# klausondrag/FOSVOS

Hardware: AMD Instinct MI355X
Metric: online fine-tune frames/sec (854x480) (higher is better)
Workload: dtype bf16; 1 GPU; OSVOS_VGG train_online one-shot fine-tune: 1x3x480x854 frame per step, fwd + class-balanced BCE + bwd, fused SGD step every 5 steps (BASELINE.json configs[1]); batch=1, avg_grad_every_n=5, activations=bf16 NHWC, fp32 accumulate, fp32 master weights, parallelism=single GPU

## Files before the change

### fosvos_amd/csrc/conv_igemm.hip

```cpp
#include <stdlib.h>

#include "common.hpp"

using namespace fosvos;

namespace {

constexpr unsigned kReluAfterAdd = 0x100u;
constexpr unsigned kSubsample2 = 0x200u;
constexpr unsigned kNoSplitK = 0x400u;

struct ConvArgs {
    const uint16_t *x;
    const uint16_t *w;
    const float *bias;
    const uint16_t *relu_src;
    const uint8_t *relu_bits;
    const uint16_t *addend;
    void *y;
    uint16_t *y_pool;
    const uint16_t *unpool_g;
    int N, H, W, Cin, Cout, Co_pad;
    int tiles_x, tiles_y;
    unsigned flags;
    int swizzle;
    int k_splits;
    int chunks_per_split;
    float *partial;
    unsigned m_ncb, m_nt, m_tx, m_ty;
    int n_t;
#ifdef FOSVOS_STAMP
    unsigned long long *stamps;
#endif
};

#ifdef FOSVOS_STAMP
unsigned long long *g_stamps = nullptr;
#define FOSVOS_STAMP_AT(i)                                                                               \
    if (a.stamps && threadIdx.x == 0)                                                                    \
        a.stamps[((((int64_t)blockIdx.z * gridDim.y + blockIdx.y) * gridDim.x + blockIdx.x) << 4) + (i)] = \
            __builtin_amdgcn_s_memtime();
#define FOSVOS_STAMP_RT(i)                                                                               \
    if (a.stamps && threadIdx.x == 0)                                                                    \
        a.stamps[((((int64_t)blockIdx.z * gridDim.y + blockIdx.y) * gridDim.x + blockIdx.x) << 4) + (i)] = \
            __builtin_amdgcn_s_memrealtime();
#else
#define FOSVOS_STAMP_AT(i)
#define FOSVOS_STAMP_RT(i)
#endif

__device__ __forceinline__ unsigned fast_div(unsigned n, unsigned d, unsigned m) { return m ? __umulhi(n, m) : n / d; }
unsigned recip_mul(int64_t n_max, int64_t d) {
    return (d >= 2 && n_max * d < (int64_t(1) << 32)) ? (unsigned)((int64_t(1) << 32) / d + 1) : 0u;
}

template <int TH_, int TW_, int BN_, int WM_, int WN_>
struct Tile {
    static constexpr int TH = TH_, TW = TW_, BN = BN_, WM = WM_, WN = WN_;
    static constexpr int BM = TH * TW;
    static constexpr int HALO_W = TW + 2, HALO_H = TH + 2;
    static constexpr int NPIX = HALO_W * HALO_H;
    static constexpr int NPIX8 = (NPIX + 7) / 8 * 8;
    static constexpr int NPIX_PAD = (NPIX + 15) / 16 * 16;
    static constexpr int WAVE_M = BM / WM, WAVE_N = BN / WN;
    static constexpr int MF = WAVE_M / 16, NF = WAVE_N / 16;
    static constexpr int A_SLOTS = 4 * NPIX_PAD;
    static constexpr int B_SLOTS = 36 * BN;
    static constexpr int NT = 64 * WM * WN;
    static constexpr int A_IT = (NPIX8 * 4 + NT - 1) / NT;
    static constexpr int B_IT = (B_SLOTS + NT - 1) / NT;
    static constexpr int OUT_LD = BN + 8;
    static constexpr int LDS_MAIN = (A_SLOTS + B_SLOTS) * 16;
    static constexpr int LDS_OUT = BM * OUT_LD * 2;
    static constexpr int LDS_BYTES = LDS_MAIN > LDS_OUT ? LDS_MAIN : LDS_OUT;
#ifndef FOSVOS_MID_WPE
#define FOSVOS_MID_WPE 3
#endif
    static constexpr int WPE = (BM >= 256 || BN < 64) ? 2 : FOSVOS_MID_WPE;
    static_assert(WM * WN == 4 || WM * WN == 8, "4 or 8 waves per workgroup");
    static_assert(TW % 16 == 0 && WAVE_M % 16 == 0 && WAVE_N % 16 == 0, "fragment alignment");
    static_assert(BM % WM == 0 && BN % WN == 0, "wave split");
};

template <int MF, int NF>
struct TapPlan {
    static constexpr int rows_b = MF / 2 > 0 ? MF / 2 : 1;
    static constexpr int per_row = (NF + rows_b - 1) / rows_b;
    static constexpr int nb(int i) {
        const int left = NF - i * per_row;
        return left <= 0 ? 0 : (left < per_row ? left : per_row);
    }
};
template <int MF, int NF, int I, bool NEXT, int V>
__device__ __forceinline__ void sched_row() {
    if constexpr (I < MF) {
        __builtin_amdgcn_sched_group_barrier(0x008, NF, 0);
        if constexpr (NEXT) __builtin_amdgcn_sched_group_barrier(0x100, 1 + TapPlan<MF, NF>::nb(I), 0);
        constexpr int rows_v = V < MF ? V : MF;
        constexpr int nv = I < MF - rows_v ? 0 : (I == MF - 1 ? V - (rows_v - 1) : 1);
        if constexpr (nv > 0) __builtin_amdgcn_sched_group_barrier(0x020, nv, 0);
    }
}
template <int MF, int NF, bool NEXT, int V>
__device__ __forceinline__ void sched_tap() {
    static_assert(MF <= 8, "sched_tap rows");
    sched_row<MF, NF, 0, NEXT, V>(); sched_row<MF, NF, 1, NEXT, V>(); sched_row<MF, NF, 2, NEXT, V>();
    sched_row<MF, NF, 3, NEXT, V>(); sched_row<MF, NF, 4, NEXT, V>(); sched_row<MF, NF, 5, NEXT, V>();
    sched_row<MF, NF, 6, NEXT, V>(); sched_row<MF, NF, 7, NEXT, V>();
}

template <class T, bool OUT_F32, bool UNPOOL = false>
__global__ __launch_bounds__(T::NT) __attribute__((amdgpu_waves_per_eu(2, T::WPE))) void k_conv3x3_igemm(const ConvArgs a) {
    extern __shared__ __attribute__((aligned(16))) uint4 smem[];
    uint4 *sA = smem;
    uint4 *sB = smem + T::A_SLOTS;
#ifdef FOSVOS_IGEMM_PRIO
    __builtin_amdgcn_s_setprio(FOSVOS_IGEMM_PRIO);
#endif

    const int tid = threadIdx.x, lane = tid & 63;
    const int wave = __builtin_amdgcn_readfirstlane(tid >> 6);
    const int wm = wave / T::WN, wn = wave % T::WN;
    int t = blockIdx.x;
    int cb = blockIdx.y;
    if (a.swizzle) {
        const int n_wg = gridDim.x, n_cb = a.Cout / T::BN, n_t = a.n_t;
        const int q8 = n_wg >> 3, r8 = n_wg & 7, xcd = t & 7;
        const int swz = (xcd < r8 ? xcd * (q8 + 1) : r8 * (q8 + 1) + (xcd - r8) * q8) + (t >> 3);
        if (a.swizzle == 1) { t = fast_div(swz, n_cb, a.m_ncb); cb = swz - t * n_cb; }
        else { cb = fast_div(swz, n_t, a.m_nt); t = swz - cb * n_t; }
    }
    const int t_row = fast_div(t, a.tiles_x, a.m_tx);
    const int tx_i = t - t_row * a.tiles_x;
    const int n = fast_div(t_row, a.tiles_y, a.m_ty);
    const int ty_i = t_row - n * a.tiles_y;
    const int y0 = ty_i * T::TH, x0 = tx_i * T::TW;
    const int n0 = cb * T::BN;
    const int H = a.H, W = a.W, Cin = a.Cin;
    const int n_chunks = Cin >> 5;
    const uint16_t *xn = a.x + (int64_t)n * H * W * Cin;

    int a_goff[T::A_IT];
    int a_slot[T::A_IT];
#pragma unroll
    for (int it = 0; it < T::A_IT; ++it) {
        const int idx = it * T::NT + tid;
        const int oct = idx >> 5, within = idx & 31;
        const int kg = within >> 3;
        const int P = oct * 8 + (within & 7);
        a_slot[it] = -1;
        a_goff[it] = -1;
        if (P < T::NPIX) {
            const int hy = P / T::HALO_W, hx = P - hy * T::HALO_W;
            const int gy = y0 + hy - 1, gx = x0 + hx - 1;
            a_slot[it] = kg * T::NPIX_PAD + P;
            if (gy >= 0 && gy < H && gx >= 0 && gx < W) a_goff[it] = ((gy * W + gx) * Cin + kg * 8) * 2;
        }
    }

    f32x4 acc[T::MF][T::NF];
#pragma unroll
    for (int i = 0; i < T::MF; ++i)
#pragma unroll
        for (int j = 0; j < T::NF; ++j) acc[i][j] = f32x4{0.f, 0.f, 0.f, 0.f};

    int a_base[T::MF];
#pragma unroll
    for (int i = 0; i < T::MF; ++i) {
        const int pb = wm * T::WAVE_M + i * 16;
        const int ty = pb / T::TW, tx = pb % T::TW;
        a_base[i] = (lane >> 4) * T::NPIX_PAD + ty * T::HALO_W + tx + (lane & 15);
    }
    const int b_base = (lane >> 4) * T::BN + wn * T::WAVE_N + (lane & 15);

    const int c_begin = a.k_splits > 1 ? blockIdx.z * a.chunks_per_split : 0;
    const int c_end = a.k_splits > 1 ? min(c_begin + a.chunks_per_split, n_chunks) : n_chunks;

    static_assert(T::A_IT <= 6 && T::B_IT <= 9, "prefetch register file");
    uint4 pa0, pa1, pa2, pa3, pa4, pa5, pb0, pb1, pb2, pb3, pb4, pb5, pb6, pb7, pb8;
    [[maybe_unused]] uint4 pa6, pa7, pa8;
    pa0 = pa1 = pa2 = pa3 = pa4 = pa5 = pb0 = pb1 = pb2 = pb3 = pb4 = pb5 = pb6 = pb7 = pb8 = make_uint4(0, 0, 0, 0);
    const int x_bytes = H * W * Cin * 2, w_bytes = (n_chunks * 36 * a.Co_pad - n0) * 16;
    auto x_rsrc = __builtin_amdgcn_make_buffer_rsrc(const_cast<uint16_t *>(xn), 0, x_bytes, 0x00020000);
    auto w_rsrc = __builtin_amdgcn_make_buffer_rsrc(const_cast<uint16_t *>(a.w) + (int64_t)n0 * 8, 0, w_bytes,
                                                    0x00020000);
    static_assert(T::NT % T::BN == 0, "weight staging assumes BN divides the workgroup size");
    const int b_voff = ((tid / T::BN) * a.Co_pad + tid % T::BN) * 16;
    const int b_row_bytes = a.Co_pad * 16;
#define FOSVOS_LD_A(i)                                                                                  \
    if constexpr (i < T::A_IT)                                                                          \
        pa##i = __builtin_bit_cast(uint4, __builtin_amdgcn_raw_buffer_load_b128(x_rsrc, a_goff[i], cc_ * 64, 0));
#define FOSVOS_LD_B(i)                                                                                  \
    if constexpr (i < T::B_IT)                                                                          \
        pb##i = __builtin_bit_cast(uint4, __builtin_amdgcn_raw_buffer_load_b128(                        \
            w_rsrc, b_voff, (cc_ * 36 + i * (T::NT / T::BN)) * b_row_bytes, 0));
#define FOSVOS_LOAD_CHUNK(cc_expr)                                                                      \
    {                                                                                                   \
        const int cc_ = (cc_expr);                                                                      \
        FOSVOS_LD_A(0) FOSVOS_LD_A(1) FOSVOS_LD_A(2) FOSVOS_LD_A(3) FOSVOS_LD_A(4) FOSVOS_LD_A(5)       \
        FOSVOS_LD_B(0) FOSVOS_LD_B(1) FOSVOS_LD_B(2) FOSVOS_LD_B(3) FOSVOS_LD_B(4) FOSVOS_LD_B(5)       \
        FOSVOS_LD_B(6) FOSVOS_LD_B(7) FOSVOS_LD_B(8)                                                    \
    }
#define FOSVOS_ST_A(i)                                                                                  \
    if constexpr (i < T::A_IT) {                                                                        \
        if (a_slot[i] >= 0) sA[a_slot[i]] = pa##i;                                                      \
    }
#define FOSVOS_ST_B(i)                                                                                  \
    if constexpr (i < T::B_IT) {                                                                        \
        if (i * T::NT + tid < T::B_SLOTS) sB[i * T::NT + tid] = pb##i;                                  \
    }
#define FOSVOS_STORE_CHUNK()                                                                            \
    {                                                                                                   \
        FOSVOS_ST_A(0) FOSVOS_ST_A(1) FOSVOS_ST_A(2) FOSVOS_ST_A(3) FOSVOS_ST_A(4) FOSVOS_ST_A(5)       \
        FOSVOS_ST_B(0) FOSVOS_ST_B(1) FOSVOS_ST_B(2) FOSVOS_ST_B(3) FOSVOS_ST_B(4) FOSVOS_ST_B(5)       \
        FOSVOS_ST_B(6) FOSVOS_ST_B(7) FOSVOS_ST_B(8)                                                    \
    }

#define FOSVOS_RD_A(tap_, i_) \
    af[i_] = __builtin_bit_cast(bf16x8, sA[a_base[i_] + ((tap_) / 3) * T::HALO_W + (tap_) % 3]);
#define FOSVOS_RD_B(tap_, buf_, j_) \
    bfr[buf_][j_] = __builtin_bit_cast(bf16x8, sB[b_base + (tap_) * 4 * T::BN + (j_) * 16]);
#define FOSVOS_ROW(tap_, i_)                                                                            \
    if constexpr ((i_) < T::MF) {                                                                       \
        _Pragma("unroll") for (int j = 0; j < T::NF; ++j) acc[i_][j] =                                  \
            __builtin_amdgcn_mfma_f32_16x16x32_bf16(bfr[(tap_) & 1][j], af[i_], acc[i_][j], 0, 0, 0);   \
        if constexpr ((tap_) < 8) {                                                                     \
            FOSVOS_RD_A((tap_) + 1, i_)                                                                 \
            _Pragma("unroll") for (int j = 0; j < TP::nb(i_); ++j)                                      \
                FOSVOS_RD_B((tap_) + 1, ((tap_) + 1) & 1, (i_) * TP::per_row + j)                       \
        }                                                                                               \
    }
#define FOSVOS_TAP(tap_)                                                                                \
    {                                                                                                   \
        FOSVOS_ROW(tap_, 0) FOSVOS_ROW(tap_, 1) FOSVOS_ROW(tap_, 2) FOSVOS_ROW(tap_, 3)                 \
        FOSVOS_ROW(tap_, 4) FOSVOS_ROW(tap_, 5) FOSVOS_ROW(tap_, 6) FOSVOS_ROW(tap_, 7)                 \
        {                                                                                               \
            const int cc_ = cc + 1;                                                                     \
            FOSVOS_LD_B(tap_)                                                                           \
            FOSVOS_LD_A(tap_)                                                                           \
        }                                                                                               \
        sched_tap<T::MF, T::NF, ((tap_) < 8), 1 + ((tap_) < T::A_IT ? 1 : 0)>();                        \
    }

    FOSVOS_STAMP_RT(11)
    FOSVOS_STAMP_AT(0)
    if (c_begin < c_end) FOSVOS_LOAD_CHUNK(c_begin)
    FOSVOS_STAMP_AT(1)
    using TP = TapPlan<T::MF, T::NF>;
    static_assert(T::MF <= 8, "row macros cover up to 8 pixel fragments per wave");
    bf16x8 af[T::MF], bfr[2][T::NF];
    for (int cc = c_begin; cc < c_end; ++cc) {
        if (cc > c_begin) __syncthreads();
        if (cc == c_end - 1) { FOSVOS_STAMP_AT(6) }
        FOSVOS_STORE_CHUNK()
        if (cc == c_begin) { FOSVOS_STAMP_AT(2) }
        if (cc == c_end - 1) { FOSVOS_STAMP_AT(7) }
        __syncthreads();
        if (cc == c_begin) { FOSVOS_STAMP_AT(3) }
#pragma unroll
        for (int i = 0; i < T::MF; ++i) FOSVOS_RD_A(0, i)
#pragma unroll
        for (int j = 0; j < T::NF; ++j) FOSVOS_RD_B(0, 0, j)
        __builtin_amdgcn_sched_group_barrier(0x100, T::MF + T::NF, 0);
        if (cc + 1 == c_end) {
            x_rsrc = __builtin_amdgcn_make_buffer_rsrc(const_cast<uint16_t *>(xn), 0, 0, 0x00020000);
            w_rsrc = __builtin_amdgcn_make_buffer_rsrc(const_cast<uint16_t *>(a.w) + (int64_t)n0 * 8, 0, 0, 0x00020000);
        }
        FOSVOS_TAP(0) FOSVOS_TAP(1) FOSVOS_TAP(2) FOSVOS_TAP(3) FOSVOS_TAP(4) FOSVOS_TAP(5) FOSVOS_TAP(6)
        FOSVOS_TAP(7) FOSVOS_TAP(8)
        if (cc == c_begin) { FOSVOS_STAMP_AT(5) }
    }
    FOSVOS_STAMP_AT(8)

    const int q = lane >> 4, cl = lane & 15;
    if (a.k_splits > 1) {
        float *po = a.partial + (int64_t)blockIdx.z * a.N * H * W * a.Cout;
#pragma unroll
        for (int i = 0; i < T::MF; ++i) {
            const int pix = wm * T::WAVE_M + i * 16 + cl;
            const int gy = y0 + pix / T::TW, gx = x0 + pix % T::TW;
            if (gy < H && gx < W) {
                float *row = po + (((int64_t)n * H + gy) * W + gx) * a.Cout + n0 + wn * T::WAVE_N + q * 4;
#pragma unroll
                for (int j = 0; j < T::NF; ++j)
                    *reinterpret_cast<float4 *>(row + j * 16) =
                        make_float4(acc[i][j][0], acc[i][j][1], acc[i][j][2], acc[i][j][3]);
            }
        }
        return;
    }
    if (OUT_F32) {
        float *yo = reinterpret_cast<float *>(a.y);
#pragma unroll
        for (int j = 0; j < T::NF; ++j) {
            const int co = n0 + wn * T::WAVE_N + j * 16 + q * 4;
            float4 b = make_float4(0.f, 0.f, 0.f, 0.f);
            if (a.bias) b = *reinterpret_cast<const float4 *>(a.bias + co);
#pragma unroll
            for (int i = 0; i < T::MF; ++i) {
                const int pix = wm * T::WAVE_M + i * 16 + cl;
                const int gy = y0 + pix / T::TW, gx = x0 + pix % T::TW;
                if (gy < H && gx < W) {
                    float4 v = make_float4(acc[i][j][0] + b.x, acc[i][j][1] + b.y, acc[i][j][2] + b.z,
                                           acc[i][j][3] + b.w);
                    if (a.flags & FOSVOS_CONV_RELU)
                        v = make_float4(relu_f(v.x), relu_f(v.y), relu_f(v.z), relu_f(v.w));
                    *reinterpret_cast<float4 *>(yo + (((int64_t)n * H + gy) * W + gx) * a.Cout + co) = v;
                }
            }
        }
        return;
    }
    constexpr int VEC_PER_PIX = T::BN / 8;
    constexpr int OUT_N = T::BM * VEC_PER_PIX;
    constexpr int OUT_IT = (OUT_N + T::NT - 1) / T::NT;
    constexpr int PIX_STEP = T::NT / VEC_PER_PIX;
    static_assert(T::NT % VEC_PER_PIX == 0 && PIX_STEP % T::TW == 0, "a thread's output vectors must share a column");
    constexpr int ROW_STEP = PIX_STEP / T::TW;
    const int o_cg = tid % VEC_PER_PIX, o_pix = tid / VEC_PER_PIX;
    const int o_ly = o_pix / T::TW, o_gx = x0 + o_pix % T::TW;
    const int img_bytes = H * W * a.Cout * 2;
    uint16_t *yo = reinterpret_cast<uint16_t *>(a.y);
    int voff[OUT_IT];
#pragma unroll
    for (int it = 0; it < OUT_IT; ++it) {
        const int gy = y0 + o_ly + it * ROW_STEP;
        const bool ok = it * T::NT + tid < OUT_N && gy < H && o_gx < W;
        voff[it] = ok ? ((gy * W + o_gx) * a.Cout + n0 + o_cg * 8) * 2 : -1;
    }
    const bool masked = (a.relu_src || a.relu_bits || a.addend) && !(a.flags & kSubsample2);
    uint4 mk[OUT_IT], ad[OUT_IT];
#pragma unroll
    for (int it = 0; it < OUT_IT; ++it) mk[it] = ad[it] = make_uint4(0, 0, 0, 0);
    if constexpr (UNPOOL) {
        const int OH = (H + 1) >> 1, OW = (W + 1) >> 1;
        auto m_rsrc = __builtin_amdgcn_make_buffer_rsrc(const_cast<uint16_t *>(a.relu_src + (int64_t)n * H * W * a.Cout), 0,
                                                        img_bytes, 0x00020000);
        auto g_rsrc = __builtin_amdgcn_make_buffer_rsrc(const_cast<uint16_t *>(a.unpool_g + (int64_t)n * OH * OW * a.Cout), 0,
                                                        OH * OW * a.Cout * 2, 0x00020000);
#pragma unroll
        for (int it = 0; it < OUT_IT; ++it)
            mk[it] = __builtin_bit_cast(uint4, __builtin_amdgcn_raw_buffer_load_b128(m_rsrc, voff[it], 0, 0));
#pragma unroll
        for (int it = 0; it < OUT_IT; ++it) {
            const int gy = y0 + o_ly + it * ROW_STEP;
            const int goff = voff[it] < 0 ? -1 : (((gy >> 1) * OW + (o_gx >> 1)) * a.Cout + n0 + o_cg * 8) * 2;
            ad[it] = __builtin_bit_cast(uint4, __builtin_amdgcn_raw_buffer_load_b128(g_rsrc, goff, 0, 0));
        }
    } else if (masked && a.relu_bits) {
        auto b_rsrc = __builtin_amdgcn_make_buffer_rsrc(const_cast<uint8_t *>(a.relu_bits + (int64_t)n * H * W * (a.Cout >> 3)), 0,
                                                        img_bytes >> 4, 0x00020000);
#pragma unroll
        for (int it = 0; it < OUT_IT; ++it) {
            const unsigned b = __builtin_amdgcn_raw_buffer_load_b8(b_rsrc, voff[it] < 0 ? -1 : voff[it] >> 4, 0, 0);
            mk[it] = make_uint4((b & 1u) | ((b & 2u) << 15), ((b >> 2) & 1u) | ((b & 8u) << 13), ((b >> 4) & 1u) | ((b & 32u) << 11),
                                ((b >> 6) & 1u) | ((b & 128u) << 9));
        }
        if (a.addend) {
            auto ad_rsrc = __builtin_amdgcn_make_buffer_rsrc(const_cast<uint16_t *>(a.addend + (int64_t)n * H * W * a.Cout), 0,
                                                             img_bytes, 0x00020000);
#pragma unroll
            for (int it = 0; it < OUT_IT; ++it)
                ad[it] = __builtin_bit_cast(uint4, __builtin_amdgcn_raw_buffer_load_b128(ad_rsrc, voff[it], 0, 0));
        }
    } else if (masked) {
        auto m_rsrc = __builtin_amdgcn_make_buffer_rsrc(
            const_cast<uint16_t *>(a.relu_src ? a.relu_src + (int64_t)n * H * W * a.Cout : yo), 0,
            a.relu_src ? img_bytes : 0, 0x00020000);
        auto ad_rsrc = __builtin_amdgcn_make_buffer_rsrc(
            const_cast<uint16_t *>(a.addend ? a.addend + (int64_t)n * H * W * a.Cout : yo), 0,
            a.addend ? img_bytes : 0, 0x00020000);
#pragma unroll
        for (int it = 0; it < OUT_IT; ++it)
            mk[it] = __builtin_bit_cast(uint4, __builtin_amdgcn_raw_buffer_load_b128(m_rsrc, voff[it], 0, 0));
#pragma unroll
        for (int it = 0; it < OUT_IT; ++it)
            ad[it] = __builtin_bit_cast(uint4, __builtin_amdgcn_raw_buffer_load_b128(ad_rsrc, voff[it], 0, 0));
    }
    float4 bias_r[T::NF];
#pragma unroll
    for (int j = 0; j < T::NF; ++j)
        bias_r[j] = a.bias ? *reinterpret_cast<const float4 *>(a.bias + n0 + wn * T::WAVE_N + j * 16 + q * 4)
                           : make_float4(0.f, 0.f, 0.f, 0.f);
    __syncthreads();
    uint16_t *sO = reinterpret_cast<uint16_t *>(smem);
#pragma unroll
    for (int j = 0; j < T::NF; ++j) {
        const int col = wn * T::WAVE_N + j * 16 + q * 4;
        const float4 b = bias_r[j];
#pragma unroll
        for (int i = 0; i < T::MF; ++i) {
            const int pix = wm * T::WAVE_M + i * 16 + cl;
            float v0 = acc[i][j][0] + b.x, v1 = acc[i][j][1] + b.y, v2 = acc[i][j][2] + b.z, v3 = acc[i][j][3] + b.w;
            if (a.flags & FOSVOS_CONV_RELU) {
                v0 = relu_f(v0); v1 = relu_f(v1); v2 = relu_f(v2); v3 = relu_f(v3);
            }
            *reinterpret_cast<uint2 *>(sO + pix * T::OUT_LD + col) = make_uint2(pack2bf(v0, v1), pack2bf(v2, v3));
        }
    }
    if constexpr (UNPOOL) {
        uint16_t *sX = sO + T::BM * T::OUT_LD;
#pragma unroll
        for (int it = 0; it < OUT_IT; ++it)
            if (it * T::NT + tid < OUT_N)
                *reinterpret_cast<uint4 *>(sX + (o_pix + it * PIX_STEP) * T::OUT_LD + o_cg * 8) = mk[it];
    }
    __syncthreads();
    FOSVOS_STAMP_AT(9)
    const uint16_t *s_vec = sO + o_pix * T::OUT_LD + o_cg * 8;
    auto y_rsrc = __builtin_amdgcn_make_buffer_rsrc(yo + (int64_t)n * H * W * a.Cout, 0, img_bytes, 0x00020000);
    if constexpr (UNPOOL) {
        static_assert((T::TW & (T::TW - 1)) == 0 && T::TH % 2 == 0, "window partners are pix ^ 1 and pix ^ TW");
        const uint16_t *sX = sO + T::BM * T::OUT_LD;
        const fosvos_i16x2 one2 = {1, 1}, zero2 = {0, 0};
        const fosvos_i16x2 late_x = (o_pix & 1) ? zero2 : one2;
#pragma unroll
        for (int it = 0; it < OUT_IT; ++it) {
            const int pix = o_pix + it * PIX_STEP;
            if (it * T::NT + tid >= OUT_N) continue;
            const fosvos_i16x2 late_y = (pix & T::TW) ? zero2 : one2;
            const uint4 cv = keep_where_pos_bf16x8(*reinterpret_cast<const uint4 *>(s_vec + it * PIX_STEP * T::OUT_LD), mk[it]);
            const uint4 x1 = *reinterpret_cast<const uint4 *>(sX + (pix ^ 1) * T::OUT_LD + o_cg * 8);
            const uint4 x2 = *reinterpret_cast<const uint4 *>(sX + (pix ^ T::TW) * T::OUT_LD + o_cg * 8);
            const uint4 x3 = *reinterpret_cast<const uint4 *>(sX + (pix ^ T::TW ^ 1) * T::OUT_LD + o_cg * 8);
            auto win = [&](unsigned own_, unsigned p1, unsigned p2, unsigned p3) {
                const fosvos_i16x2 own = __builtin_bit_cast(fosvos_i16x2, own_);
                const fosvos_i16x2 s = (zero2 - own) & (__builtin_bit_cast(fosvos_i16x2, p1) - own - late_x) &
                                       (__builtin_bit_cast(fosvos_i16x2, p2) - own - late_y) &
                                       (__builtin_bit_cast(fosvos_i16x2, p3) - own - late_y);
                return __builtin_bit_cast(unsigned, s >> 15);
            };
            const uint4 routed = make_uint4(ad[it].x & win(mk[it].x, x1.x, x2.x, x3.x), ad[it].y & win(mk[it].y, x1.y, x2.y, x3.y),
                                            ad[it].z & win(mk[it].z, x1.z, x2.z, x3.z), ad[it].w & win(mk[it].w, x1.w, x2.w, x3.w));
            float f[8], r[8];
            unpack8(cv, f);
            unpack8(routed, r);
#pragma unroll
            for (int e = 0; e < 8; ++e) f[e] += r[e];
            __builtin_amdgcn_raw_buffer_store_b128(__builtin_bit_cast(u32x4, pack8(f)), y_rsrc, voff[it], 0, 0);
        }
    } else if (!(a.flags & kSubsample2)) {
        if (masked) {
#pragma unroll
            for (int it = 0; it < OUT_IT; ++it) {
                uint4 v = *reinterpret_cast<const uint4 *>(s_vec + it * PIX_STEP * T::OUT_LD);
                if (a.relu_src || a.relu_bits) v = keep_where_pos_bf16x8(v, mk[it]);
                if (a.addend || (a.flags & kReluAfterAdd)) {
                    float f[8];
                    unpack8(v, f);
                    if (a.addend) {
                        float av[8];
                        unpack8(ad[it], av);
#pragma unroll
                        for (int e = 0; e < 8; ++e) f[e] += av[e];
                    }
                    if (a.flags & kReluAfterAdd) {
#pragma unroll
                        for (int e = 0; e < 8; ++e) f[e] = relu_f(f[e]);
                    }
                    v = pack8(f);
                }
                __builtin_amdgcn_raw_buffer_store_b128(__builtin_bit_cast(u32x4, v), y_rsrc, voff[it], 0, 0);
            }
        } else {
#pragma unroll
            for (int it = 0; it < OUT_IT; ++it)
                __builtin_amdgcn_raw_buffer_store_b128(
                    __builtin_bit_cast(u32x4, *reinterpret_cast<const uint4 *>(s_vec + it * PIX_STEP * T::OUT_LD)), y_rsrc,
                    voff[it], 0, 0);
        }
    } else {
#pragma unroll
        for (int it = 0; it < OUT_IT; ++it) {
            const int gy = y0 + o_ly + it * ROW_STEP;
            if (it * T::NT + tid >= OUT_N || gy >= H || o_gx >= W || ((gy | o_gx) & 1)) continue;
            const int64_t off =
                (((int64_t)n * ((H + 1) >> 1) + (gy >> 1)) * ((W + 1) >> 1) + (o_gx >> 1)) * a.Cout + n0 + o_cg * 8;
            *reinterpret_cast<uint4 *>(yo + off) = *reinterpret_cast<const uint4 *>(s_vec + it * PIX_STEP * T::OUT_LD);
        }
    }
    if (a.y_pool) {
        static_assert(T::TH % 2 == 0 && T::TW % 2 == 0, "pooling windows must not straddle tiles");
        constexpr int PW = T::TW / 2, PN = (T::TH / 2) * PW;
        const int OH = (H + 1) >> 1, OW = (W + 1) >> 1;
        auto p_rsrc = __builtin_amdgcn_make_buffer_rsrc(a.y_pool + (int64_t)n * OH * OW * a.Cout, 0, OH * OW * a.Cout * 2,
                                                        0x00020000);
        for (int idx = tid; idx < PN * VEC_PER_PIX; idx += T::NT) {
            const int pp = idx / VEC_PER_PIX, cg = idx % VEC_PER_PIX;
            const int py = pp / PW, px = pp % PW;
            const int oy = (y0 >> 1) + py, ox = (x0 >> 1) + px;
            if (oy >= OH || ox >= OW) continue;
            const int poff = ((oy * OW + ox) * a.Cout + n0 + cg * 8) * 2;
// ... 91 lines not shown
            }
            if (a.addend) {
                float ad[8];
                unpack8(*reinterpret_cast<const uint4 *>(a.addend + off), ad);
#pragma unroll
                for (int e = 0; e < 8; ++e) f[e] += ad[e];
            }
            if (a.flags & kReluAfterAdd) {
#pragma unroll
                for (int e = 0; e < 8; ++e) f[e] = relu_f(f[e]);
            }
        }
        *reinterpret_cast<uint4 *>(reinterpret_cast<uint16_t *>(a.y) + i * 8) = pack8(f);
    }
}

using TileBig = Tile<8, 32, 64, 4, 1>;
using TileSquare = Tile<16, 16, 64, 4, 1>;
using TileMid = Tile<8, 16, 64, 2, 2>;
using TileSmall = Tile<4, 16, 64, 2, 2>;
using TileSide = Tile<8, 32, 16, 4, 1>;
using TileSideS = Tile<4, 16, 16, 4, 1>;
using TileHalf = Tile<8, 32, 32, 4, 1>;
using TileHalfS = Tile<4, 16, 32, 4, 1>;

enum TileId { kBig, kMid, kSmall, kSide, kSideS, kHalf, kHalfS, kSquare };

struct ConvPlan {
    TileId tile;
    int k_splits, chunks_per_split;
    size_t workspace_bytes;
};

constexpr int kMinBlocks = 512;

ConvPlan make_plan(int N, int H, int W, int in_ch, int out_ch) {
    ConvPlan p{};
    const int n_chunks = roundup(in_ch, 32) / 32;
    const int64_t pixels = (int64_t)N * H * W;
    auto blocks = [&](int th, int tw, int bn) { return cdiv(W, tw) * cdiv(H, th) * N * (int64_t)(out_ch / bn); };
    int64_t nb;
    if (out_ch % 64 == 0) {
        bool big = blocks(8, 32, 64) >= kMinBlocks / 2;
        if (big) {
            const int64_t area_wide = cdiv(H, 8) * 8 * cdiv(W, 32) * 32, area_sq = cdiv(H, 16) * 16 * cdiv(W, 16) * 16;
            static const bool allow_sq = lab_env_int("FOSVOS_NO_SQUARE_TILE", 0) == 0;
            if (allow_sq && area_sq < area_wide) { p.tile = kSquare; nb = blocks(16, 16, 64); }
            else { p.tile = kBig; nb = blocks(8, 32, 64); }
            static const bool one_round = lab_env_int("FOSVOS_MID_ONE_ROUND", 0) != 0;
            if (blocks(8, 16, 64) <= 768 && (one_round ? blocks(8, 32, 64) < kMinBlocks * 3 / 4 : nb < kMinBlocks / 2)) big = false;
        }
        if (!big) { p.tile = kMid; nb = blocks(8, 16, 64); }
    } else if (out_ch == 32) {
        if (pixels >= 256 * 256) { p.tile = kHalf; nb = blocks(8, 32, 32); }
        else { p.tile = kHalfS; nb = blocks(4, 16, 32); }
    } else {
        if (pixels >= 256 * 256) { p.tile = kSide; nb = blocks(8, 32, 16); }
        else { p.tile = kSideS; nb = blocks(4, 16, 16); }
    }
    if (out_ch % 64 == 0) {
        static const char *force = lab_env("FOSVOS_FORCE_TILE");
        if (force && ((atoi(force) >= 0 && atoi(force) <= 2) || atoi(force) == (int)kHalf)) {
            p.tile = (TileId)atoi(force);
            nb = p.tile == kBig ? blocks(8, 32, 64) : p.tile == kMid ? blocks(8, 16, 64)
                 : p.tile == kHalf ? blocks(8, 32, 32) : blocks(4, 16, 64);
        }
    }
    int ks = 1;
    if (nb < kMinBlocks * 3 / 4) {
        ks = (int)cdiv(kMinBlocks / 2, nb);
        if (ks < 2) ks = 1;
        if (ks > n_chunks) ks = n_chunks;
        if (ks > 16) ks = 16;
    }
#ifdef FOSVOS_STAMP
    if (const char *e = lab_env("FOSVOS_FORCE_KS")) ks = atoi(e);
#endif
    p.chunks_per_split = (int)cdiv(n_chunks, ks);
    p.k_splits = (int)cdiv(n_chunks, p.chunks_per_split);
    p.workspace_bytes = p.k_splits > 1 ? (size_t)p.k_splits * pixels * out_ch * sizeof(float) : 0;
    return p;
}

template <class T, bool OUT_F32, bool UNPOOL = false>
int launch(const ConvArgs &a0, const ConvPlan &plan, hipStream_t st, int in_ch) {
    constexpr int LDS = UNPOOL && 2 * T::LDS_OUT > T::LDS_MAIN ? 2 * T::LDS_OUT : T::LDS_BYTES;
    ConvArgs a = a0;
    a.tiles_x = (int)cdiv(a.W, T::TW);
    a.tiles_y = (int)cdiv(a.H, T::TH);
    a.k_splits = plan.k_splits;
    a.chunks_per_split = plan.chunks_per_split;
#ifdef FOSVOS_STAMP
    a.stamps = g_stamps;
#endif
    const int64_t tiles = (int64_t)a.tiles_x * a.tiles_y * a.N;
    FOSVOS_REQUIRE(tiles <= 0x7fffffff && a.Cout % T::BN == 0, FOSVOS_E_SHAPE, "conv3x3: tile grid");
    if constexpr (LDS > 64 * 1024) {
        static bool once[64];
        int dev = 0;
        FOSVOS_HIP_CHECK(hipGetDevice(&dev));
        if (dev >= 0 && dev < 64 && !once[dev]) {
            FOSVOS_HIP_CHECK(hipFuncSetAttribute(reinterpret_cast<const void *>(k_conv3x3_igemm<T, OUT_F32, UNPOOL>),
                                                 hipFuncAttributeMaxDynamicSharedMemorySize, LDS));
            once[dev] = true;
        }
    }
    if (g_prof_on) {
        static char name[80];
        snprintf(name, sizeof(name), "k_conv3x3_igemm<Tile<%d, %d, %d, %d, %d>, %s, %s>", T::TH, T::TW, T::BN, T::WM, T::WN,
                 OUT_F32 ? "true" : "false", UNPOOL ? "true" : "false");
        prof_begin(name, st, 2.0 * a.N * a.H * a.W * 9.0 * in_ch * a.Cout);
    }
    {
        static const int swz_env = lab_env_int("FOSVOS_IGEMM_SWIZZLE", -1);
        const int n_cb = a.Cout / T::BN;
        a.swizzle = swz_env >= 0 ? swz_env : (tiles * n_cb >= 64 ? 1 : 0);
        if (tiles * n_cb > 0x7fffffff) a.swizzle = 0;
    }
    {
        const int64_t n_cb = a.Cout / T::BN, n_wg = tiles * n_cb;
        a.n_t = (int)tiles;
        a.m_ncb = recip_mul(n_wg, n_cb);
        a.m_nt = recip_mul(n_wg, tiles);
        a.m_tx = recip_mul(tiles, a.tiles_x);
        a.m_ty = recip_mul(tiles, a.tiles_y);
    }
    const dim3 grid = a.swizzle ? dim3((unsigned)(tiles * (a.Cout / T::BN)), 1u, (unsigned)plan.k_splits)
                                : dim3((unsigned)tiles, (unsigned)(a.Cout / T::BN), (unsigned)plan.k_splits);
    hipLaunchKernelGGL((k_conv3x3_igemm<T, OUT_F32, UNPOOL>), grid, dim3(T::NT), LDS, st, a);
    FOSVOS_LAUNCH_CHECK();
    if (plan.k_splits > 1) {
        const int64_t total8 = (a.flags & kSubsample2) ? (int64_t)a.N * ((a.H + 1) >> 1) * ((a.W + 1) >> 1) * (a.Cout / 8)
                                                       : (int64_t)a.N * a.H * a.W * (a.Cout / 8);
        int64_t g = cdiv(total8, 256);
        if (g > 4096) g = 4096;
        FOSVOS_PROF("k_splitk_epilogue", st, 0.0);
        hipLaunchKernelGGL(k_splitk_epilogue, dim3((unsigned)g), dim3(256), 0, st, a, total8);
        FOSVOS_LAUNCH_CHECK();
    }
    return FOSVOS_OK;
}

int dispatch(ConvArgs a, int in_ch, void *workspace, size_t workspace_bytes, hipStream_t st) {
    const bool f32 = (a.flags & FOSVOS_CONV_OUT_F32) != 0;
    if (a.Cout == 32) {
        FOSVOS_REQUIRE(!f32, FOSVOS_E_ARG, "conv3x3: fp32 output is only built for 16-channel outputs");
    } else if (a.Cout % 64 != 0) {
        FOSVOS_REQUIRE(a.Cout == 16, FOSVOS_E_SHAPE, "conv3x3: output channels must be 16, 32 or a multiple of 64 (got %d)",
                       a.Cout);
        FOSVOS_REQUIRE(a.relu_src == nullptr && a.addend == nullptr, FOSVOS_E_ARG,
                       "conv3x3: 16-channel output has no mask/add epilogue");
    } else {
        FOSVOS_REQUIRE(!f32, FOSVOS_E_ARG, "conv3x3: fp32 output is only built for 16-channel outputs");
    }
    ConvPlan plan = make_plan(a.N, a.H, a.W, in_ch, a.Cout);
    if (a.flags & kNoSplitK) {
        plan.k_splits = 1;
        plan.chunks_per_split = roundup(in_ch, 32) / 32;
        plan.workspace_bytes = 0;
    }
    if (plan.k_splits > 1) {
        FOSVOS_REQUIRE(workspace && workspace_bytes >= plan.workspace_bytes, FOSVOS_E_WORKSPACE,
                       "conv3x3: split-K needs %zu workspace bytes, got %zu", plan.workspace_bytes, workspace_bytes);
        a.partial = reinterpret_cast<float *>(workspace);
    }
    if (a.unpool_g) {
        switch (plan.tile) {
            case kBig: return launch<TileBig, false, true>(a, plan, st, in_ch);
            case kSquare: return launch<TileSquare, false, true>(a, plan, st, in_ch);
            case kMid: return launch<TileMid, false, true>(a, plan, st, in_ch);
            default: return fail(FOSVOS_E_ARG, "conv3x3: no fused pool backward for this tile");
        }
    }
    switch (plan.tile) {
        case kBig: return launch<TileBig, false>(a, plan, st, in_ch);
        case kSquare: return launch<TileSquare, false>(a, plan, st, in_ch);
        case kMid: return launch<TileMid, false>(a, plan, st, in_ch);
        case kSmall: return launch<TileSmall, false>(a, plan, st, in_ch);
        case kSide: return f32 ? launch<TileSide, true>(a, plan, st, in_ch) : launch<TileSide, false>(a, plan, st, in_ch);
        case kSideS: return f32 ? launch<TileSideS, true>(a, plan, st, in_ch) : launch<TileSideS, false>(a, plan, st, in_ch);
        case kHalf: return launch<TileHalf, false>(a, plan, st, in_ch);
        case kHalfS: return launch<TileHalfS, false>(a, plan, st, in_ch);
    }
    return fail(FOSVOS_E_ARG, "conv3x3: bad plan");
}

bool forward_takes_pp(int N, int H, int W, int in_ch, int out_ch, unsigned flags) {
    if (flags & ~FOSVOS_CONV_RELU) return false;
    static const int mode = lab_env_int("FOSVOS_PP", -1);
    if (mode == 0) return false;
    return conv_pp_applicable(N, H, W, roundup(in_ch, 32), out_ch);
}

int check_common(const void *x, const void *w, const void *y, int N, int H, int W, int in_ch, int out_ch,
                 const char *who) {
    FOSVOS_REQUIRE(x && w && y, FOSVOS_E_ARG, "%s: null pointer", who);
    FOSVOS_REQUIRE(N > 0 && H > 0 && W > 0 && in_ch > 0 && out_ch > 0, FOSVOS_E_SHAPE, "%s: bad shape N=%d H=%d W=%d in=%d out=%d",
                   who, N, H, W, in_ch, out_ch);
    FOSVOS_REQUIRE(out_ch % 16 == 0, FOSVOS_E_SHAPE, "%s: output channels %d not a multiple of 16", who, out_ch);
    FOSVOS_REQUIRE((int64_t)H * W * roundup(in_ch, 32) * 2 < 0x7fffffffLL && (int64_t)H * W * out_ch * 4 < 0x7fffffffLL,
                   FOSVOS_E_SHAPE, "%s: one image exceeds 2^31 bytes", who);
    return FOSVOS_OK;
}
}

extern "C" size_t fosvos_conv3x3_workspace_bytes(int N, int H, int W, int in_ch, int out_ch) {
    if (N <= 0 || H <= 0 || W <= 0 || in_ch <= 0 || out_ch <= 0 || (out_ch % 64 != 0 && out_ch != 16)) return 0;
    return make_plan(N, H, W, in_ch, out_ch).workspace_bytes;
}

extern "C" int fosvos_conv3x3_plan(int N, int H, int W, int in_ch, int out_ch, fosvos_conv3x3_plan_info *out) {
    FOSVOS_REQUIRE(out, FOSVOS_E_ARG, "conv3x3_plan: null output");
    FOSVOS_REQUIRE(N > 0 && H > 0 && W > 0 && in_ch > 0 && out_ch > 0 && (out_ch % 64 == 0 || out_ch == 32 || out_ch == 16),
                   FOSVOS_E_SHAPE, "conv3x3_plan: bad shape N=%d H=%d W=%d in=%d out=%d", N, H, W, in_ch, out_ch);
    const ConvPlan p = make_plan(N, H, W, in_ch, out_ch);
    int th = 0, tw = 0, bn = 0;
    switch (p.tile) {
        case kBig: th = TileBig::TH; tw = TileBig::TW; bn = TileBig::BN; break;
        case kSquare: th = TileSquare::TH; tw = TileSquare::TW; bn = TileSquare::BN; break;
        case kMid: th = TileMid::TH; tw = TileMid::TW; bn = TileMid::BN; break;
        case kSmall: th = TileSmall::TH; tw = TileSmall::TW; bn = TileSmall::BN; break;
        case kSide: th = TileSide::TH; tw = TileSide::TW; bn = TileSide::BN; break;
        case kSideS: th = TileSideS::TH; tw = TileSideS::TW; bn = TileSideS::BN; break;
        case kHalf: th = TileHalf::TH; tw = TileHalf::TW; bn = TileHalf::BN; break;
        case kHalfS: th = TileHalfS::TH; tw = TileHalfS::TW; bn = TileHalfS::BN; break;
    }
    out->tile_h = th; out->tile_w = tw; out->tile_co = bn;
    out->k_splits = p.k_splits;
    out->workgroups = (int)(cdiv(W, tw) * cdiv(H, th) * N * (out_ch / bn));
    out->persistent = 0;
    return FOSVOS_OK;
}

extern "C" int fosvos_conv3x3_fwd_plan(int N, int H, int W, int in_ch, int out_ch, unsigned flags,
                                       fosvos_conv3x3_plan_info *out) {
    if (int rc = fosvos_conv3x3_plan(N, H, W, in_ch, out_ch, out)) return rc;
    if (out_ch % 64 == 0 && forward_takes_pp(N, H, W, in_ch, out_ch, flags)) {
        out->tile_h = 8; out->tile_w = 32; out->tile_co = 64;
        out->k_splits = 1;
        out->workgroups = conv_pp_workgroups();
        out->persistent = 1;
    }
    return FOSVOS_OK;
}

extern "C" int fosvos_conv3x3_fwd(const uint16_t *x, const uint16_t *w_packed, const float *bias, void *y, int N, int H,
                                  int W, int Ci, int Co, unsigned flags, void *workspace, size_t workspace_bytes,
// ... 52 lines not shown
    FOSVOS_REQUIRE(Co % 64 == 0, FOSVOS_E_SHAPE, "conv3x3_fwd_pool: Co=%d must be a multiple of 64", Co);
    if ((flags & FOSVOS_CONV_RELU) && forward_takes_pp(N, H, W, Ci, Co, flags)) {
        FOSVOS_ENTER(device);
        return conv_pp_forward(x, w_packed, bias, y, y_pool, N, H, W, roundup(Ci, 32), Co, roundup(Co, 16), true,
                               (hipStream_t)stream);
    }
    if (make_plan(N, H, W, Ci, Co).k_splits > 1) {
        if (int rc = fosvos_conv3x3_fwd(x, w_packed, bias, y, N, H, W, Ci, Co, flags, workspace, workspace_bytes, device, stream))
            return rc;
        return fosvos_maxpool2x2_ceil_fwd(y, y_pool, N, H, W, Co, device, stream);
    }
    FOSVOS_ENTER(device);
    ConvArgs a{};
    a.x = x; a.w = w_packed; a.bias = bias; a.relu_src = nullptr; a.addend = nullptr; a.y = y; a.y_pool = y_pool;
    a.N = N; a.H = H; a.W = W; a.Cin = roundup(Ci, 32); a.Cout = Co; a.Co_pad = roundup(Co, 16); a.flags = flags;
    return dispatch(a, Ci, workspace, workspace_bytes, (hipStream_t)stream);
}

namespace fosvos {
bool conv3x3_pool_codes_applicable(int N, int H, int W, int Ci, int Co) {
    if (N <= 0 || H <= 0 || W <= 0 || Ci <= 0 || Co <= 0 || Co % 64 != 0) return false;
    if ((int64_t)H * W * roundup(Ci, 32) * 2 >= 0x7fffffffLL || (int64_t)H * W * Co * 4 >= 0x7fffffffLL) return false;
    return forward_takes_pp(N, H, W, Ci, Co, FOSVOS_CONV_RELU);
}
}

extern "C" size_t fosvos_conv3x3_pool_codes_bytes(int N, int H, int W, int C) {
    if (N <= 0 || H <= 0 || W <= 0 || C <= 0 || C % 8 != 0) return 0;
    return (size_t)N * ((H + 1) / 2) * ((W + 1) / 2) * (C / 8) * 4;
}

extern "C" int fosvos_conv3x3_fwd_pool_codes(const uint16_t *x, const uint16_t *w_packed, const float *bias,
                                             uint16_t *y_pool, uint32_t *codes, int N, int H, int W, int Ci, int Co,
                                             unsigned flags, int device, void *stream) {
    if (int rc = check_common(x, w_packed, y_pool, N, H, W, Ci, Co, "conv3x3_fwd_pool_codes")) return rc;
    FOSVOS_REQUIRE(codes, FOSVOS_E_ARG, "conv3x3_fwd_pool_codes: null codes output");
    FOSVOS_REQUIRE(((uintptr_t)codes & 3) == 0, FOSVOS_E_ARG, "conv3x3_fwd_pool_codes: codes must be 4-byte aligned");
    FOSVOS_REQUIRE(flags == FOSVOS_CONV_RELU, FOSVOS_E_ARG,
                   "conv3x3_fwd_pool_codes: flags 0x%x (the codes are taken on post-ReLU values: FOSVOS_CONV_RELU)", flags);
    FOSVOS_REQUIRE(Co % 64 == 0, FOSVOS_E_SHAPE, "conv3x3_fwd_pool_codes: Co=%d must be a multiple of 64", Co);
    FOSVOS_REQUIRE(conv3x3_pool_codes_applicable(N, H, W, Ci, Co), FOSVOS_E_SHAPE,
                   "conv3x3_fwd_pool_codes: N=%d H=%d W=%d Ci=%d Co=%d is not a shape of the persistent kernel (use "
                   "fosvos_conv3x3_fwd_pool)", N, H, W, Ci, Co);
    FOSVOS_ENTER(device);
    return conv_pp_forward(x, w_packed, bias, nullptr, y_pool, N, H, W, roundup(Ci, 32), Co, roundup(Co, 16), true,
                           (hipStream_t)stream, nullptr, codes);
}

extern "C" int fosvos_conv3x3_dgrad_bits(const uint16_t *dy, const uint16_t *w_dgrad_packed, const uint8_t *relu_bits,
                                         const uint16_t *addend, uint16_t *dx, int N, int H, int W, int Ci, int Co,
                                         void *workspace, size_t workspace_bytes, int device, void *stream) {
    if (int rc = check_common(dy, w_dgrad_packed, dx, N, H, W, Co, Ci, "conv3x3_dgrad_bits")) return rc;
    FOSVOS_REQUIRE(relu_bits && Ci % 8 == 0, FOSVOS_E_ARG, "conv3x3_dgrad_bits: null mask or Ci=%d not a multiple of 8", Ci);
    FOSVOS_ENTER(device);
    if (!addend && lab_env_int("FOSVOS_PP_DGRAD", 1) != 0 && lab_env_int("FOSVOS_PP", -1) != 0 &&
        conv_pp_applicable(N, H, W, roundup(Co, 32), Ci))
        return conv_pp_forward(dy, w_dgrad_packed, nullptr, dx, nullptr, N, H, W, roundup(Co, 32), Ci, roundup(Ci, 16), false,
                               (hipStream_t)stream, relu_bits);
    ConvArgs a{};
    a.x = dy; a.w = w_dgrad_packed; a.bias = nullptr; a.relu_src = nullptr; a.relu_bits = relu_bits; a.addend = addend; a.y = dx;
    a.N = N; a.H = H; a.W = W; a.Cin = roundup(Co, 32); a.Cout = Ci; a.Co_pad = roundup(Ci, 16); a.flags = 0;
    return dispatch(a, Co, workspace, workspace_bytes, (hipStream_t)stream);
}

extern "C" int fosvos_conv3x3_dgrad_unpool(const uint16_t *dy, const uint16_t *w_dgrad_packed, const uint16_t *x,
                                           const uint16_t *d_pooled, uint16_t *dx, int N, int H, int W, int Ci, int Co,
                                           void *workspace, size_t workspace_bytes, int device, void *stream) {
    if (int rc = check_common(dy, w_dgrad_packed, dx, N, H, W, Co, Ci, "conv3x3_dgrad_unpool")) return rc;
    FOSVOS_REQUIRE(x && d_pooled && x != dx, FOSVOS_E_ARG, "conv3x3_dgrad_unpool: null or aliased pooled-map operands");
    FOSVOS_ENTER(device);
    const ConvPlan plan = make_plan(N, H, W, Co, Ci);
    const bool fused = Ci % 64 == 0 && plan.k_splits == 1 && (plan.tile == kBig || plan.tile == kSquare || plan.tile == kMid) &&
                       lab_env_int("FOSVOS_UNPOOL_FUSED", 1) != 0;
    if (!fused) {
        if (int rc = fosvos_maxpool2x2_ceil_bwd(x, d_pooled, dx, N, H, W, Ci, 1, device, stream)) return rc;
        return fosvos_conv3x3_dgrad(dy, w_dgrad_packed, x, dx, dx, N, H, W, Ci, Co, workspace, workspace_bytes, device, stream);
    }
    ConvArgs a{};
    a.x = dy; a.w = w_dgrad_packed; a.relu_src = x; a.unpool_g = d_pooled; a.y = dx;
    a.N = N; a.H = H; a.W = W; a.Cin = roundup(Co, 32); a.Cout = Ci; a.Co_pad = roundup(Ci, 16); a.flags = 0;
    return dispatch(a, Co, workspace, workspace_bytes, (hipStream_t)stream);
}

extern "C" int fosvos_conv3x3_dgrad(const uint16_t *dy, const uint16_t *w_dgrad_packed, const uint16_t *relu_src,
                                    const uint16_t *addend, uint16_t *dx, int N, int H, int W, int Ci, int Co,
                                    void *workspace, size_t workspace_bytes, int device, void *stream) {
    if (int rc = check_common(dy, w_dgrad_packed, dx, N, H, W, Co, Ci, "conv3x3_dgrad")) return rc;
    FOSVOS_ENTER(device);
    ConvArgs a{};
    a.x = dy; a.w = w_dgrad_packed; a.bias = nullptr; a.relu_src = relu_src; a.addend = addend; a.y = dx;
    a.N = N; a.H = H; a.W = W; a.Cin = roundup(Co, 32); a.Cout = Ci; a.Co_pad = roundup(Ci, 16); a.flags = 0;
    return dispatch(a, Co, workspace, workspace_bytes, (hipStream_t)stream);
}
```

### fosvos_amd/csrc/vgg_net.hip

```cpp
#include <stdlib.h>

#include "common.hpp"

using namespace fosvos;

namespace {
constexpr int kNConv = 13;
constexpr int kStageOf[kNConv] = {0, 0, 1, 1, 2, 2, 2, 3, 3, 3, 4, 4, 4};
constexpr int kCin[kNConv] = {3, 64, 64, 128, 128, 256, 256, 256, 512, 512, 512, 512, 512};
constexpr int kCout[kNConv] = {64, 64, 128, 128, 256, 256, 256, 512, 512, 512, 512, 512, 512};
constexpr int kFirstOfStage[5] = {0, 2, 4, 7, 10};
constexpr int kLastOfStage[5] = {1, 3, 6, 9, 12};
constexpr int kStageCh[5] = {64, 128, 256, 512, 512};

inline size_t up256(size_t v) { return (v + 255) / 256 * 256; }

struct Arena {
    int sh[5], sw[5];
    size_t act[kNConv];
    size_t gact[kNConv];
    size_t pooled[4];
    size_t gpooled[4];
    size_t side[4];
    size_t dside[4];
// ... 237 lines not shown
            if (c == kFirstOfStage[s])
                x = reinterpret_cast<uint16_t *>(base + a.pooled[s - 1]);
            if (c == 1 && compact) {
                FOSVOS_TRY(fosvos_conv3x3_fwd_pool_codes(x, w->conv_wf[c], w->conv_b[c], reinterpret_cast<uint16_t *>(base + a.pooled[0]),
                                                         codes1(0), N, H, W, kCin[c], kCout[c], FOSVOS_CONV_RELU, device, stream));
            } else if (c == kLastOfStage[s] && s < 4) {
                FOSVOS_TRY(fosvos_conv3x3_fwd_pool(x, w->conv_wf[c], w->conv_b[c], act(c),
                                                   reinterpret_cast<uint16_t *>(base + a.pooled[s]), N, a.sh[s], a.sw[s],
                                                   kCin[c], kCout[c], FOSVOS_CONV_RELU, ws, a.ws_bytes, device, stream));
            } else {
                FOSVOS_TRY(fosvos_conv3x3_fwd(x, w->conv_wf[c], w->conv_b[c], act(c), N, a.sh[s], a.sw[s], kCin[c], kCout[c],
                                              FOSVOS_CONV_RELU, ws, a.ws_bytes, device, stream));
            }
        }
        x = act(c);
        if (s > 0 && c == kLastOfStage[s]) {
            const bool on_aux = par && s < 4;
            if (on_aux) {
                FOSVOS_HIP_CHECK(hipEventRecord(ev[c], sm));
                FOSVOS_HIP_CHECK(hipStreamWaitEvent(sa, ev[c], 0));
            }
            FOSVOS_TRY(fosvos_conv3x3_fwd(x, w->side_wf[s - 1], w->side_b[s - 1], base + a.side[s - 1], N, a.sh[s], a.sw[s],
                                          kStageCh[s], 16, FOSVOS_CONV_OUT_F32, on_aux ? base + a.wsa_side[s - 1] : ws,
                                          on_aux ? a.wsa_side_bytes[s - 1] : a.ws_bytes, device, on_aux ? sa : sm));
        }
    }
    if (par) {
        FOSVOS_HIP_CHECK(hipEventRecord(ev[13], sa));
        FOSVOS_HIP_CHECK(hipStreamWaitEvent(sm, ev[13], 0));
    }
    }
    const float *side[4];
    int hs[4], wsz[4];
    for (int i = 0; i < 4; ++i) {
        side[i] = reinterpret_cast<const float *>(base + a.side[i]);
        hs[i] = a.sh[i + 1];
        wsz[i] = a.sw[i + 1];
    }
    return fosvos_head_fwd(side, hs, wsz, w->filt, w->filt1, w->dsn_w, w->dsn_b, w->fuse_w, w->fuse_b, fused, side_out, N, H,
                           W, w->filt_uniform, device, stream);
}
}

extern "C" int fosvos_vgg_forward_streams(fosvos_ctx *ctx, const fosvos_vgg_weights *w, const float *frame, int N, int H,
                                          int W, void *arena, size_t arena_bytes, float *fused, float *const side_out[4],
                                          void *stream, void *aux_stream) {
    return fosvos_vgg_forward_streams_flags(ctx, w, frame, N, H, W, arena, arena_bytes, fused, side_out, stream, aux_stream, 0u);
}

extern "C" int fosvos_vgg_forward_streams_flags(fosvos_ctx *ctx, const fosvos_vgg_weights *w, const float *frame, int N, int H,
                                                int W, void *arena, size_t arena_bytes, float *fused, float *const side_out[4],
                                                void *stream, void *aux_stream, unsigned flags) {
    FOSVOS_TRY(ctx_check(ctx, "vgg_forward_streams"));
    return forward_impl(ctx->vgg_ev, w, frame, N, H, W, arena, arena_bytes, fused, side_out, ctx->device, stream, aux_stream,
                        flags);
}

extern "C" int fosvos_vgg_stage1_compact(unsigned flags, int N, int H, int W) { return stage1_compact(flags, N, H, W) ? 1 : 0; }

extern "C" int fosvos_vgg_forward(const fosvos_vgg_weights *w, const float *frame, int N, int H, int W, void *arena,
                                  size_t arena_bytes, float *fused, float *const side_out[4], int device,
                                  void *stream) {
    return forward_impl(nullptr, w, frame, N, H, W, arena, arena_bytes, fused, side_out, device, stream, nullptr, 0u);
}

extern "C" int fosvos_vgg_forward_flags(const fosvos_vgg_weights *w, const float *frame, int N, int H, int W, void *arena,
                                        size_t arena_bytes, float *fused, float *const side_out[4], int device, void *stream,
                                        unsigned flags) {
    return forward_impl(nullptr, w, frame, N, H, W, arena, arena_bytes, fused, side_out, device, stream, nullptr, flags);
}

extern "C" int fosvos_vgg_backward(fosvos_ctx *ctx, const fosvos_vgg_weights *w, const fosvos_vgg_grads *g,
                                   const float *frame, int N, int H, int W, void *arena, size_t arena_bytes,
                                   const float *d_fused, const float *const d_side_out[4], void *stream,
                                   void *aux_stream) {
    return fosvos_vgg_backward_flags(ctx, w, g, frame, N, H, W, arena, arena_bytes, d_fused, d_side_out, stream, aux_stream, 0u);
}

extern "C" int fosvos_vgg_backward_flags(fosvos_ctx *ctx, const fosvos_vgg_weights *w, const fosvos_vgg_grads *g,
                                         const float *frame, int N, int H, int W, void *arena, size_t arena_bytes,
                                         const float *d_fused, const float *const d_side_out[4], void *stream,
                                         void *aux_stream, unsigned flags) {
    FOSVOS_TRY(ctx_check(ctx, "vgg_backward"));
    FOSVOS_REQUIRE((flags & ~FOSVOS_VGG_COMPACT_STAGE1) == 0, FOSVOS_E_ARG, "vgg_backward: unknown flags 0x%x", flags);
    const bool compact = stage1_compact(flags, N, H, W);
    const int device = ctx->device;
    const Arena a = make_arena(N, H, W);
    FOSVOS_TRY(check_net(w, frame, arena, N, H, W, arena_bytes, a, "vgg_backward"));
    FOSVOS_REQUIRE(g, FOSVOS_E_ARG, "vgg_backward: null gradient table");
    const bool with_so = d_side_out && d_side_out[0];
    FOSVOS_REQUIRE(d_fused || with_so, FOSVOS_E_ARG, "vgg_backward: no upstream gradient given");
    char *base = reinterpret_cast<char *>(arena);
    auto act = [&](int c) { return reinterpret_cast<uint16_t *>(base + a.act[c]); };
    auto gact = [&](int c) { return reinterpret_cast<uint16_t *>(base + a.gact[c]); };
    void *ws = base + a.ws;
    const int acc = g->accumulate ? 1 : 0;
    WgradReduceTable reduce;
    reduce.n = 0;
    WgradReduceTable reduce_m;
    reduce_m.n = 0;

    hipStream_t sm = (hipStream_t)stream;
    const bool par = aux_stream != nullptr && aux_stream != stream;
    hipStream_t sa = par ? (hipStream_t)aux_stream : sm;
    hipEvent_t *ev = ctx->vgg_ev;
    const bool buckets = g->bucket_events != 0;
    const bool tail = g->last_pass_of_cycle != 0;
    static const int tail_stages = lab_env_int("FOSVOS_TAIL_STAGES", 1);
    static const bool offload_on = lab_env_int("FOSVOS_TAIL_OFFLOAD", 1) != 0;
    const bool offload = tail && aux_stream != nullptr && aux_stream != stream && offload_on;
    FOSVOS_ENTER(device);
    ctx->buckets_recorded = false;
    if (par) {
        FOSVOS_HIP_CHECK(hipEventRecord(ev[14], sm));
        FOSVOS_HIP_CHECK(hipStreamWaitEvent(sa, ev[14], 0));
    }
    auto publish = [&](int e) -> int {
        if (!par) return FOSVOS_OK;
        FOSVOS_HIP_CHECK(hipEventRecord(ev[e], sm));
        FOSVOS_HIP_CHECK(hipStreamWaitEvent(sa, ev[e], 0));
        return FOSVOS_OK;
    };

    const float *side[4];
    uint16_t *dside[4];
    int hs[4], wsz[4];
    for (int i = 0; i < 4; ++i) {
        side[i] = reinterpret_cast<const float *>(base + a.side[i]);
        dside[i] = reinterpret_cast<uint16_t *>(base + a.dside[i]);
        hs[i] = a.sh[i + 1];
        wsz[i] = a.sw[i + 1];
    }
    const HeadBwdArgs ha{side, hs, wsz, w->filt, with_so ? w->filt1 : nullptr, with_so ? w->dsn_w : nullptr, w->fuse_w,
                         d_fused, with_so ? d_side_out : nullptr, dside, g->fuse_w, g->fuse_b,
                         with_so ? g->dsn_w : nullptr, with_so ? g->dsn_b : nullptr, N, H, W, acc, base + a.hws,
                         a.hws_bytes, device, w->filt_uniform & 15};
    FOSVOS_TRY(head_bwd_check(ha));
    FOSVOS_TRY(head_bwd_scale(ha, 3, sm));
    for (int i = 2; i >= 0; --i) {
        FOSVOS_TRY(head_bwd_scale(ha, i, sa));
        if (par) FOSVOS_HIP_CHECK(hipEventRecord(ev[16 + i], sa));
    }
    FOSVOS_TRY(publish(13));
    FOSVOS_TRY(head_bwd_finish(ha, sa));

    static const bool unpool_fused = lab_env_int("FOSVOS_UNPOOL", 1) != 0;
    for (int s = 4; s >= 0; --s) {
        const int hh = a.sh[s], ww = a.sw[s], last = kLastOfStage[s], first = kFirstOfStage[s];
        if (s > 0) {
            FOSVOS_TRY(wgrad_impl(act(last), dside[s - 1], g->side_w[s - 1], g->side_b[s - 1], N, hh, ww, kStageCh[s], 16,
                                  acc, base + a.wsa_side[s - 1], a.wsa_side_bytes[s - 1], device, sa,
                                  (offload && s == 1) ? &reduce_m : &reduce, tail && s <= tail_stages));
            const uint16_t *addend = (s < 4) ? gact(last) : nullptr;
            if (par && s < 4) FOSVOS_HIP_CHECK(hipStreamWaitEvent(sm, ev[16 + s - 1], 0));
            if (s < 4 && unpool_fused)
                FOSVOS_TRY(fosvos_conv3x3_dgrad_unpool(dside[s - 1], w->side_wd[s - 1], act(last),
                                                       reinterpret_cast<const uint16_t *>(base + a.gpooled[s]), gact(last), N, hh,
                                                       ww, kStageCh[s], 16, ws, a.ws_bytes, device, sm));
            else
                FOSVOS_TRY(fosvos_conv3x3_dgrad(dside[s - 1], w->side_wd[s - 1], act(last), addend, gact(last), N, hh, ww,
                                                kStageCh[s], 16, ws, a.ws_bytes, device, sm));
        }
        FOSVOS_TRY(publish(last));
        for (int c = last; c >= first; --c) {
            if (c == 0) {
                if (offload)
                    FOSVOS_TRY(first_wgrad_impl(frame, gact(0), g->conv_w[0], g->conv_b[0], N, H, W, kCout[0], acc,
                                                base + a.wsa_conv[0], a.wsa_conv_bytes[0], device, sm, &reduce_m));
                else
                    FOSVOS_TRY(first_wgrad_impl(frame, gact(0), g->conv_w[0], g->conv_b[0], N, H, W, kCout[0], acc,
                                                base + a.wsa_conv[0], a.wsa_conv_bytes[0], device, sa, &reduce));
                break;
            }
            const bool from_pool = (c == first) && s > 0;
            const uint16_t *xin = from_pool ? reinterpret_cast<const uint16_t *>(base + a.pooled[s - 1]) : act(c - 1);
            uint16_t *dx = from_pool ? reinterpret_cast<uint16_t *>(base + a.gpooled[s - 1]) : gact(c - 1);
            const uint16_t *mask = from_pool ? nullptr : act(c - 1);
            const bool middle = (last - first == 2) && c == last - 1;
            if (!middle)
                FOSVOS_TRY(wgrad_impl(xin, gact(c), g->conv_w[c], g->conv_b[c], N, hh, ww, kCin[c], kCout[c], acc,
                                      base + a.wsa_conv[c], a.wsa_conv_bytes[c], device, sa,
                                      (offload && s == 1) ? &reduce_m : &reduce, tail && s <= tail_stages));
            static const bool bits_on = lab_env_int("FOSVOS_RELU_BITS", 1) != 0;
            if (c == 1 && bits_on)
                FOSVOS_TRY(fosvos_conv3x3_dgrad_bits(gact(c), w->conv_wd[c], reinterpret_cast<const uint8_t *>(base + a.bits0), nullptr,
                                                     dx, N, hh, ww, kCin[c], kCout[c], ws, a.ws_bytes, device, sm));
            else
                FOSVOS_TRY(fosvos_conv3x3_dgrad(gact(c), w->conv_wd[c], mask, nullptr, dx, N, hh, ww, kCin[c], kCout[c], ws,
                                                a.ws_bytes, device, sm));
            const bool skip_event = (last - first == 2) && c == last;
            if (!from_pool && !skip_event) FOSVOS_TRY(publish(c - 1));
            if (middle)
                FOSVOS_TRY(wgrad_impl(xin, gact(c), g->conv_w[c], g->conv_b[c], N, hh, ww, kCin[c], kCout[c], acc,
                                      base + a.wsa_conv[c], a.wsa_conv_bytes[c], device, sa,
                                      (offload && s == 1) ? &reduce_m : &reduce, tail && s <= tail_stages));
        }
        if (s == 1 && compact)
            FOSVOS_TRY(fosvos_maxpool2x2_ceil_bwd_codes(reinterpret_cast<const uint32_t *>(base + a.act[1]),
                                                        reinterpret_cast<const uint16_t *>(base + a.gpooled[0]), gact(1), N, a.sh[0],
                                                        a.sw[0], kStageCh[0], device, sm));
        else if (s == 1 || (s > 0 && !unpool_fused))
            FOSVOS_TRY(fosvos_maxpool2x2_ceil_bwd(act(kLastOfStage[s - 1]), reinterpret_cast<const uint16_t *>(base + a.gpooled[s - 1]),
                                                  gact(kLastOfStage[s - 1]), N, a.sh[s - 1], a.sw[s - 1], kStageCh[s - 1], 1,
                                                  device, sm));
        if (s >= 1) {
            FOSVOS_TRY(wgrad_reduce_all(&reduce, device, sa));
            if (buckets && s >= 2) FOSVOS_HIP_CHECK(hipEventRecord(ev[kBucketEvent0 + (4 - s)], sa));
            if (offload && s == 1) FOSVOS_HIP_CHECK(hipEventRecord(ev[kStage2WgradEvent], sa));
        }
    }
    FOSVOS_TRY(wgrad_reduce_all(&reduce, device, sa));
    if (offload) {
        FOSVOS_HIP_CHECK(hipStreamWaitEvent(sm, ev[kStage2WgradEvent], 0));
        FOSVOS_TRY(wgrad_reduce_all(&reduce_m, device, sm));
    }
    if (buckets) FOSVOS_HIP_CHECK(hipEventRecord(ev[kMainTailEvent], sm));
    if (buckets) {
        FOSVOS_HIP_CHECK(hipEventRecord(ev[kBucketFinalEvent], sa));
        ctx->buckets_recorded = true;
    }
    if (par && !g->defer_join) {
        FOSVOS_HIP_CHECK(hipEventRecord(ev[15], sa));
        FOSVOS_HIP_CHECK(hipStreamWaitEvent(sm, ev[15], 0));
    }
    return FOSVOS_OK;
}

extern "C" int fosvos_vgg_grad_bucket_wait(fosvos_ctx *ctx, int bucket, void *stream) {
    FOSVOS_TRY(ctx_check(ctx, "vgg_grad_bucket_wait"));
    FOSVOS_REQUIRE(bucket >= 0 && bucket < 5, FOSVOS_E_ARG, "vgg_grad_bucket_wait: bucket %d not in 0..4", bucket);
    FOSVOS_ENTER(ctx->device);
    FOSVOS_REQUIRE(ctx->buckets_recorded, FOSVOS_E_ARG,
                   "vgg_grad_bucket_wait: the last fosvos_vgg_backward on this context did not set grads.bucket_events");
    hipEvent_t *ev = ctx->vgg_ev;
    if (bucket < 3) {
        FOSVOS_HIP_CHECK(hipStreamWaitEvent((hipStream_t)stream, ev[kBucketEvent0 + bucket], 0));
    } else {
        FOSVOS_HIP_CHECK(hipStreamWaitEvent((hipStream_t)stream, ev[kBucketFinalEvent], 0));
        FOSVOS_HIP_CHECK(hipStreamWaitEvent((hipStream_t)stream, ev[kMainTailEvent], 0));
    }
    return FOSVOS_OK;
}
```

### fosvos_amd/fosvos_hip/__init__.py

```python
from __future__ import annotations

import ctypes
import os
import threading
from ctypes import POINTER, c_char_p, c_float, c_int, c_int64, c_size_t, c_uint, c_void_p

_HERE = os.path.dirname(os.path.abspath(__file__))
PKG_ROOT = os.path.dirname(_HERE)
LIB_PATH = os.environ.get("FOSVOS_HIP_LIB") or os.path.join(PKG_ROOT, "lib", "libfosvos_hip.so")
HEADER_PATH = os.path.join(os.path.dirname(PKG_ROOT), "include", "fosvos_hip.h")

ABI_VERSION = 33
CONV_RELU = 1
CONV_OUT_F32 = 2
VGG_COMPACT_STAGE1 = 1


class FosvosHipError(RuntimeError):
    pass


class SgdEntry(ctypes.Structure):
    _fields_ = [("param", c_void_p), ("grad", c_void_p), ("momentum_buf", c_void_p), ("numel", c_int64),
                ("lr", c_float), ("weight_decay", c_float)]


_P4 = c_void_p * 4
_I4 = c_int * 4
_P13 = c_void_p * 13


class VggWeights(ctypes.Structure):
    _fields_ = [("conv_w", _P13), ("conv_b", _P13), ("conv_wf", _P13), ("conv_wd", _P13),
                ("side_b", _P4), ("side_wf", _P4), ("side_wd", _P4), ("filt", _P4), ("filt1", _P4),
                ("dsn_w", c_void_p), ("dsn_b", c_void_p), ("fuse_w", c_void_p), ("fuse_b", c_void_p),
                ("filt_uniform", c_int)]


class VggGrads(ctypes.Structure):
    _fields_ = [("conv_w", _P13), ("conv_b", _P13), ("side_w", _P4), ("side_b", _P4),
                ("dsn_w", c_void_p), ("dsn_b", c_void_p), ("fuse_w", c_void_p), ("fuse_b", c_void_p),
                ("accumulate", c_int), ("defer_join", c_int), ("bucket_events", c_int), ("last_pass_of_cycle", c_int)]

_Z4 = c_size_t * 4
_Z13 = c_size_t * 13


class VggArenaLayout(ctypes.Structure):
    _fields_ = [("total", c_size_t), ("stage_h", c_int * 5), ("stage_w", c_int * 5),
                ("act", _Z13), ("gact", _Z13), ("act_bytes", _Z13),
                ("pooled", _Z4), ("gpooled", _Z4), ("pooled_bytes", _Z4),
                ("side", _Z4), ("side_bytes", _Z4), ("dside", _Z4), ("dside_bytes", _Z4),
                ("bits0", c_size_t), ("bits0_bytes", c_size_t),
                ("ws", c_size_t), ("ws_bytes", c_size_t), ("hws", c_size_t), ("hws_bytes", c_size_t),
                ("wsa_conv", _Z13), ("wsa_conv_bytes", _Z13), ("wsa_side", _Z4), ("wsa_side_bytes", _Z4)]


class Conv3x3PlanInfo(ctypes.Structure):
    _fields_ = [("tile_h", c_int), ("tile_w", c_int), ("tile_co", c_int), ("k_splits", c_int), ("workgroups", c_int),
                ("persistent", c_int)]


class Conv2dPlanInfo(ctypes.Structure):
    _fields_ = [("cob", c_int), ("threads", c_int), ("slices", c_int), ("workgroups", c_int), ("mfma_frag_blocks", c_int),
                ("mfma_workgroups", c_int)]


class ProfileRecord(ctypes.Structure):
    _fields_ = [("name", ctypes.c_char * 96), ("launches", c_int), ("ms", ctypes.c_double), ("flops", ctypes.c_double)]


class PackEntry(ctypes.Structure):
    _fields_ = [("w", c_void_p), ("w_fwd", c_void_p), ("w_dgrad", c_void_p), ("Co", c_int), ("Ci", c_int)]



class Conv2dDesc(ctypes.Structure):
    _fields_ = [("w_packed", c_void_p), ("bias", c_void_p), ("Ci", c_int), ("Co", c_int), ("k", c_int), ("stride", c_int),
                ("kind", c_int)]


class ResnetBlock(ctypes.Structure):
    _fields_ = [("conv", Conv2dDesc * 3), ("n_convs", c_int), ("has_down", c_int), ("down", Conv2dDesc)]


class ResnetNet(ctypes.Structure):
    _fields_ = [("first_w", c_void_p), ("first_b", c_void_p), ("first_co", c_int), ("first_fp32_math", c_int), ("first_unfused", c_int),
                ("blocks_per_stage", c_int * 4),
                ("blocks", POINTER(ResnetBlock)), ("side", Conv2dDesc * 4), ("filt", c_void_p * 4),
                ("filt1", c_void_p * 4), ("stride", c_int * 4), ("dsn_w", c_void_p), ("dsn_b", c_void_p),
                ("fuse_b", c_void_p)]

SIGNATURES = {
    "fosvos_abi_version": (c_int, []),
    "fosvos_last_error": (c_char_p, []),
    "fosvos_build_arch": (c_char_p, []),
    "fosvos_ctx_create": (c_int, [c_int, POINTER(c_void_p)]),
    "fosvos_ctx_destroy": (c_int, [c_void_p]),
# ... 67 lines not shown
                                      c_float, c_void_p, c_void_p, c_int, c_void_p]),
    "fosvos_conv2d_plan": (c_int, [c_int, c_int, c_int, c_int, c_int, c_int, c_int, POINTER(Conv2dPlanInfo)]),
    "fosvos_conv2d_fwd": (c_int, [c_void_p, c_void_p, c_void_p, c_void_p, c_void_p, c_int, c_int, c_int, c_int, c_int,
                                  c_int, c_int, c_uint, c_int, c_void_p]),
    "fosvos_conv7x7_packed_elems": (c_size_t, [c_int]),
    "fosvos_pack_conv7x7_bn": (c_int, [c_void_p, c_int, c_void_p, c_void_p, c_void_p, c_void_p, c_float, c_void_p,
                                       c_void_p, c_int, c_void_p]),
    "fosvos_conv7x7s2_first_fwd": (c_int, [c_void_p, c_void_p, c_void_p, c_void_p, c_int, c_int, c_int, c_int, c_uint,
                                           c_int, c_void_p]),
    "fosvos_conv7x7s2_pool_first_fwd": (c_int, [c_void_p, c_void_p, c_void_p, c_void_p, c_int, c_int, c_int, c_int, c_int,
                                                c_void_p]),
    "fosvos_maxpool3x3s2_fwd": (c_int, [c_void_p, c_void_p, c_int, c_int, c_int, c_int, c_int, c_void_p]),
    "fosvos_deconv_head_fwd": (c_int, [POINTER(c_void_p), POINTER(c_int), POINTER(c_int), POINTER(c_int),
                                       POINTER(c_void_p), POINTER(c_void_p), c_void_p, c_void_p, c_void_p, c_void_p,
                                       POINTER(c_void_p), c_int, c_int, c_int, c_int, c_void_p]),
    "fosvos_resnet_arena_bytes": (c_size_t, [POINTER(ResnetNet), c_int, c_int, c_int]),
    "fosvos_resnet_forward": (c_int, [POINTER(ResnetNet), c_void_p, c_int, c_int, c_int, c_void_p, c_size_t, c_void_p,
                                      POINTER(c_void_p), c_int, c_void_p, c_void_p, c_void_p]),
    "fosvos_vgg_arena_bytes": (c_size_t, [c_int, c_int, c_int]),
    "fosvos_vgg_arena_layout": (c_int, [c_int, c_int, c_int, POINTER(VggArenaLayout)]),
    "fosvos_vgg_grad_bucket_wait": (c_int, [c_void_p, c_int, c_void_p]),
    "fosvos_profile_start": (c_int, [c_int, c_int]),
    "fosvos_profile_stop": (c_int, [c_int, POINTER(ProfileRecord), c_int, POINTER(c_int)]),
    "fosvos_vgg_forward": (c_int, [POINTER(VggWeights), c_void_p, c_int, c_int, c_int, c_void_p, c_size_t, c_void_p,
                                   POINTER(c_void_p), c_int, c_void_p]),
    "fosvos_vgg_forward_streams": (c_int, [c_void_p, POINTER(VggWeights), c_void_p, c_int, c_int, c_int, c_void_p, c_size_t,
                                           c_void_p, POINTER(c_void_p), c_void_p, c_void_p]),
    "fosvos_augment_sample": (c_int, [c_void_p, c_void_p, c_int, c_int, c_int, c_void_p, c_void_p, c_void_p, c_void_p,
                                      c_void_p, c_void_p, c_int, c_int, c_void_p, c_void_p, c_void_p, c_void_p, c_int,
                                      c_void_p]),
    "fosvos_prob_bytes": (c_int, [c_void_p, c_int, c_int, c_int, c_void_p, c_void_p, c_int, c_void_p]),
    "fosvos_jf_workspace_bytes": (c_size_t, [c_int, c_int, c_int]),
    "fosvos_jf_counts": (c_int, [c_void_p, c_void_p, c_int, c_int, c_int, c_int, c_void_p, c_void_p, c_size_t, c_int,
                                 c_void_p]),
    "fosvos_png_capacity_bytes": (c_size_t, [c_int, c_int, c_int]),
    "fosvos_png_workspace_bytes": (c_size_t, [c_int, c_int, c_int, c_int]),
    "fosvos_png_encode": (c_int, [c_void_p, c_int, c_int, c_int, c_int, c_void_p, c_size_t, c_void_p, c_void_p, c_size_t, c_int,
                                  c_void_p]),
    "fosvos_merge_objects": (c_int, [POINTER(c_void_p), c_int, c_int, c_int, c_int, c_void_p, c_int, c_void_p]),
    "fosvos_jf_labels_workspace_bytes": (c_size_t, [c_int, c_int, c_int, c_int]),
    "fosvos_jf_counts_labels": (c_int, [c_void_p, c_void_p, c_int, c_int, c_int, c_int, c_int, c_void_p, c_void_p, c_size_t,
                                        c_int, c_void_p]),
    "fosvos_components_workspace_bytes": (c_size_t, [c_int, c_int, c_int]),
    "fosvos_component_roots": (c_int, [c_void_p, c_int, c_int, c_int, c_void_p, c_void_p, c_size_t, c_int, c_void_p]),
    "fosvos_clean_components": (c_int, [c_void_p, c_void_p, c_int, c_int, c_int, c_int, c_int, c_int, c_int, c_float, c_void_p,
                                        c_void_p, c_void_p, c_size_t, c_int, c_void_p]),
    "fosvos_cbce_void_workspace_bytes": (c_size_t, [c_int64, c_int]),
    "fosvos_cbce_loss_frames_void": (c_int, [c_void_p, c_void_p, c_void_p, c_int64, c_int, c_int, c_float, c_void_p, c_void_p,
                                             c_void_p, c_size_t, c_int, c_void_p]),
    "fosvos_distance_gate_workspace_bytes": (c_size_t, [c_int, c_int, c_int]),
    "fosvos_distance_gate": (c_int, [c_void_p, c_int, c_int, c_int, c_int, c_int, c_void_p, c_void_p, c_size_t, c_int,
                                     c_void_p]),
    "fosvos_adapt_labels_workspace_bytes": (c_size_t, [c_int, c_int, c_int]),
    "fosvos_adapt_labels": (c_int, [c_void_p, c_void_p, c_int, c_int, c_int, c_float, c_int, c_int, c_void_p, c_void_p,
                                    c_void_p, c_void_p, c_size_t, c_int, c_void_p]),
    "fosvos_png_indexed_capacity_bytes": (c_size_t, [c_int, c_int, c_int]),
    "fosvos_png_encode_indexed": (c_int, [c_void_p, c_void_p, c_int, c_int, c_int, c_int, c_void_p, c_size_t, c_void_p,
                                          c_void_p, c_size_t, c_int, c_void_p]),
    "fosvos_jpeg_capacity_bytes": (c_size_t, [c_int, c_int, c_int, c_int, c_int]),
    "fosvos_jpeg_workspace_bytes": (c_size_t, [c_int, c_int, c_int, c_int, c_int]),
    "fosvos_jpeg_encode": (c_int, [c_void_p, c_int, c_int, c_int, c_int, c_int, c_int, c_void_p, c_size_t, c_void_p, c_void_p,
                                   c_size_t, c_int, c_void_p]),
    "fosvos_jpeg_decode_workspace_bytes": (c_size_t, [c_int, c_int, c_int, c_int, c_int]),
    "fosvos_jpeg_decode": (c_int, [c_void_p, c_size_t, c_void_p, c_int, c_void_p, c_int, c_int, c_int, c_int, c_int, c_void_p,
                                   c_void_p, c_void_p, c_size_t, c_int, c_void_p]),
    "fosvos_frame_prep": (c_int, [c_void_p, c_int, c_int, c_int, c_int, POINTER(c_float), c_void_p, c_int, c_void_p]),
    "fosvos_overlay": (c_int, [c_void_p, c_void_p, c_int, c_int, c_int, c_int, c_int, c_int, ctypes.c_double, c_void_p, c_int,
                               c_void_p]),
    "fosvos_frame_prep_scaled": (c_int, [c_void_p, c_int, c_int, c_int, c_int, c_int, c_int, POINTER(c_float), c_void_p, c_int,
                                         c_void_p]),
    "fosvos_overlay_scaled": (c_int, [c_void_p, c_void_p, c_int, c_int, c_int, c_int, c_int, c_int, c_int, c_int,
                                      ctypes.c_double, c_void_p, c_int, c_void_p]),
    "fosvos_overlay_objects": (c_int, [c_void_p, POINTER(c_void_p), c_int, c_int, c_int, c_int, c_int, c_void_p,
                                       ctypes.c_double, c_void_p, c_int, c_void_p]),
    "fosvos_overlay_objects_scaled": (c_int, [c_void_p, POINTER(c_void_p), c_int, c_int, c_int, c_int, c_int, c_int, c_int,
                                              c_int, c_void_p, ctypes.c_double, c_void_p, c_int, c_void_p]),
    "fosvos_vgg_backward": (c_int, [c_void_p, POINTER(VggWeights), POINTER(VggGrads), c_void_p, c_int, c_int, c_int, c_void_p,
                                    c_size_t, c_void_p, POINTER(c_void_p), c_void_p, c_void_p]),
    "fosvos_conv3x3_fwd_pool_codes": (c_int, [c_void_p, c_void_p, c_void_p, c_void_p, c_void_p, c_int, c_int, c_int, c_int,
                                              c_int, c_uint, c_int, c_void_p]),
    "fosvos_conv3x3_pool_codes_bytes": (c_size_t, [c_int, c_int, c_int, c_int]),
    "fosvos_maxpool2x2_ceil_bwd_codes": (c_int, [c_void_p, c_void_p, c_void_p, c_int, c_int, c_int, c_int, c_int, c_void_p]),
    "fosvos_vgg_stage1_compact": (c_int, [c_uint, c_int, c_int, c_int]),
    "fosvos_vgg_forward_flags": (c_int, [POINTER(VggWeights), c_void_p, c_int, c_int, c_int, c_void_p, c_size_t, c_void_p,
                                         POINTER(c_void_p), c_int, c_void_p, c_uint]),
    "fosvos_vgg_forward_streams_flags": (c_int, [c_void_p, POINTER(VggWeights), c_void_p, c_int, c_int, c_int, c_void_p,
                                                 c_size_t, c_void_p, POINTER(c_void_p), c_void_p, c_void_p, c_uint]),
    "fosvos_vgg_backward_flags": (c_int, [c_void_p, POINTER(VggWeights), POINTER(VggGrads), c_void_p, c_int, c_int, c_int,
                                          c_void_p, c_size_t, c_void_p, POINTER(c_void_p), c_void_p, c_void_p, c_uint]),
}

_lib = None
_lock = threading.Lock()


def lib() -> ctypes.CDLL:
    global _lib
    if _lib is not None:
        return _lib
    with _lock:
        if _lib is not None:
            return _lib
        if not os.path.exists(LIB_PATH):
            raise FosvosHipError(
                f"{LIB_PATH} not found: build it with `python -c 'import __graft_entry__ as g; g.build()'` "
                f"or `make -C fosvos_amd/csrc`.  There is no CPU fallback.")
        import torch
        handle = ctypes.CDLL(LIB_PATH)
        for name, (restype, argtypes) in SIGNATURES.items():
            fn = getattr(handle, name)
            fn.restype = restype
            fn.argtypes = argtypes
        got = handle.fosvos_abi_version()
        if got != ABI_VERSION:
            raise FosvosHipError(f"libfosvos_hip.so ABI {got} != binding ABI {ABI_VERSION}: rebuild")
        _lib = handle
    return _lib


def check(rc: int, what: str) -> None:
    if rc != 0:
        msg = lib().fosvos_last_error()
        raise FosvosHipError(f"{what} failed (code {rc}): {msg.decode(errors='replace') if msg else ''}")


class LaunchProfile:

    def __init__(self, device: int, max_launches: int = 65536):
        self.device, self.max_launches, self.records = int(device), int(max_launches), {}

    def __enter__(self):
        check(lib().fosvos_profile_start(self.device, self.max_launches), "profile_start")
        return self

    def __exit__(self, *exc):
        buf = (ProfileRecord * 128)()
        n = c_int(0)
        check(lib().fosvos_profile_stop(self.device, buf, 128, ctypes.byref(n)), "profile_stop")
        self.records = {buf[i].name.decode(): {"launches": buf[i].launches, "ms": buf[i].ms, "flops": buf[i].flops}
                        for i in range(n.value)}
        return False


class Context:

    def __init__(self, device: int):
        h = c_void_p()
        check(lib().fosvos_ctx_create(int(device), ctypes.byref(h)), "ctx_create")
        self.handle, self.device = h, int(device)

    def close(self) -> None:
        h, self.handle = self.handle, None
        if h is not None and _lib is not None:
            _lib.fosvos_ctx_destroy(h)

    def __del__(self):
        try:
            self.close()
        except Exception:
            pass


def ptr_array4(ptrs) -> "ctypes.Array":
    return _P4(*[c_void_p(p) for p in ptrs])


# ... 3 lines not shown
```

### fosvos_amd/fosvos_hip/engine.py

```python
from __future__ import annotations

import ctypes
import time
from dataclasses import dataclass
from typing import Dict, List, Optional, Sequence, Tuple

import torch

from . import VGG_COMPACT_STAGE1, Context, VggGrads, VggWeights, check, lib, ops, ptr_array4
from .options import EngineOptions, native_loop_from_env

STAGE_CHANNELS = ((64, 64), (128, 128), (256, 256, 256), (512, 512, 512), (512, 512, 512))
STAGE_IN = (3, 64, 128, 256, 512)
SIDE_CH = 16


def conv_module_index(stage: int, k: int) -> int:
    return 2 * k + (0 if stage == 0 else 1)


def param_names() -> List[str]:
    names = [f"upscale.{i}.weight" for i in range(4)] + [f"upscale_.{i}.weight" for i in range(4)]
    for s, chans in enumerate(STAGE_CHANNELS):
        for j in range(len(chans)):
            m = conv_module_index(s, j)
            names += [f"stages.{s}.{m}.weight", f"stages.{s}.{m}.bias"]
    for i in range(4):
        names += [f"side_prep.{i}.weight", f"side_prep.{i}.bias"]
    for i in range(4):
        names += [f"score_dsn.{i}.weight", f"score_dsn.{i}.bias"]
    names += ["fuse.weight", "fuse.bias"]
    return names


PARAM_NAMES = param_names()
PARAM_INDEX = {n: i for i, n in enumerate(PARAM_NAMES)}


class _PassFlagsSlots:
    __slots__ = ("_compact_stage1",)


@dataclass(slots=True)
class PassFlags(_PassFlagsSlots):

    defer_wgrad_join: bool = False
    forward_one_stream: bool = False
    publish_grad_buckets: bool = False
    overwrite_grads: bool = False
    last_pass_of_cycle: bool = False

    @property
    def compact_stage1(self) -> bool:
        return getattr(self, "_compact_stage1", False)

    @compact_stage1.setter
    def compact_stage1(self, value: bool) -> None:
        self._compact_stage1 = bool(value)


class PackedWeights:

    def __init__(self, options: Optional[EngineOptions] = None) -> None:
        self.options = options if options is not None else EngineOptions.from_env()
        self.flags = PassFlags()
        self._cache: Dict[str, Tuple[object, object, object]] = {}
        self._uniform: Dict[str, bool] = {}
        self.arenas = ArenaPool()

    @staticmethod
    def _key(t: torch.Tensor) -> Tuple[int, int]:
        return (t.data_ptr(), t._version)

    def invalidate(self) -> None:
        self._cache.clear()
        self._uniform.clear()

    def small(self, name: str, parts: Sequence[torch.Tensor]) -> torch.Tensor:
        key = tuple(self._key(t) for t in parts)
        hit = self._cache.get(name)
        if hit is not None and hit[0] == key:
            return hit[1]
        cat = torch.cat([t.detach().reshape(-1) for t in parts]).contiguous()
        self._cache[name] = (key, cat, tuple(t.untyped_storage() for t in parts))
        return cat

    def conv(self, name: str, w: torch.Tensor):
        key = self._key(w)
        hit = self._cache.get(name)
        if hit is not None and hit[0] == key:
            return hit[1]
        packed = ops.pack_conv3x3_weights(w.detach(), True, True)
        self._cache[name] = (key, packed, w.untyped_storage())
        return packed

    def conv_many(self, named: Sequence[Tuple[str, torch.Tensor]]):
        stale = []
        for name, w in named:
            hit = self._cache.get(name)
            if hit is None or hit[0] != self._key(w):
                stale.append((name, w))
        if stale:
            packed = ops.pack_conv3x3_weights_multi([w.detach() for _, w in stale])
            for (name, w), pk in zip(stale, packed):
                self._cache[name] = (self._key(w), pk, w.untyped_storage())
        return [self._cache[name][1] for name, _ in named]

    def deconv_diag(self, name: str, w: torch.Tensor) -> torch.Tensor:
        key = self._key(w)
        hit = self._cache.get(name)
        if hit is not None and hit[0] == key:
            return hit[1]
        wd = w.detach()
        c = wd.shape[0]
        idx = torch.arange(c, device=wd.device)
        diag = wd[idx, idx]
        if c > 1:
            off = torch.count_nonzero(wd) - torch.count_nonzero(diag)
            if int(off) != 0:
                raise NotImplementedError(
                    f"{name}: transposed-conv weight has off-diagonal (cross-channel) entries; the HIP head "
                    f"implements the per-channel (diagonal) form the reference initialises and freezes")
        diag = diag.permute(1, 2, 0).contiguous()
        self._cache[name] = (key, diag, w.untyped_storage())
        self._uniform[name] = bool((diag == diag[..., :1]).all().item())
        return diag

    def head_uniform_mask(self, P: Dict[str, torch.Tensor]) -> int:
        if not self.options.head_uniform:
            return 0
        mask = 0
        for i in range(4):
            name = f"upscale.{i}.weight"
            self.deconv_diag(name, P[name])
            if self._uniform.get(name, False):
                mask |= 1 << i
        return mask


def _conv_list():
    out = []
# ... 258 lines not shown
        self._pending.append((n, h, w, arena, frame))

    def join(self) -> None:
        for idx, st in self._aux.items():
            torch.cuda.current_stream(idx).wait_stream(st)
        for n, h, w, arena, _frame in self._pending:
            self.give(n, h, w, arena)
        self._pending.clear()

    def give(self, n: int, h: int, w: int, arena: torch.Tensor) -> None:
        key = self._home.get(arena.data_ptr(), (n, h, w, arena.device.index))
        free = self._free.setdefault(key, [])
        if len(free) < 6:
            free.append(arena)
        else:
            self._home.pop(arena.data_ptr(), None)


def _aligned_ptr(arena: torch.Tensor) -> Tuple[int, int]:
    p = arena.data_ptr()
    ap = (p + 255) // 256 * 256
    return ap, arena.numel() - (ap - p)


def _weights_struct(P: Dict[str, torch.Tensor], packs: PackedWeights):
    w = VggWeights()
    keep = []
    named = [(wn, P[wn]) for c, (wn, _) in enumerate(_CONV_NAMES) if c > 0]
    named += [(f"side_prep.{i}.weight", P[f"side_prep.{i}.weight"]) for i in range(4)]
    images = packs.conv_many(named)
    for c, (wn, bn) in enumerate(_CONV_NAMES):
        w.conv_w[c] = P[wn].data_ptr()
        w.conv_b[c] = P[bn].data_ptr()
        if c > 0:
            wf, wd = images[c - 1]
            w.conv_wf[c], w.conv_wd[c] = wf.data_ptr(), wd.data_ptr()
    for i in range(4):
        wf, wd = images[len(_CONV_NAMES) - 1 + i]
        w.side_wf[i], w.side_wd[i] = wf.data_ptr(), wd.data_ptr()
        w.side_b[i] = P[f"side_prep.{i}.bias"].data_ptr()
        f = packs.deconv_diag(f"upscale.{i}.weight", P[f"upscale.{i}.weight"])
        f1 = packs.deconv_diag(f"upscale_.{i}.weight", P[f"upscale_.{i}.weight"])
        w.filt[i], w.filt1[i] = f.data_ptr(), f1.data_ptr()
    dsn_w = packs.small("dsn_w", [P[f"score_dsn.{i}.weight"] for i in range(4)])
    dsn_b = packs.small("dsn_b", [P[f"score_dsn.{i}.bias"] for i in range(4)])
    w.dsn_w, w.dsn_b = dsn_w.data_ptr(), dsn_b.data_ptr()
    w.fuse_w, w.fuse_b = P["fuse.weight"].data_ptr(), P["fuse.bias"].data_ptr()
    w.filt_uniform = packs.head_uniform_mask(P)
    keep += [dsn_w, dsn_b]
    return w, keep


def native_forward(P, packs, pool: ArenaPool, x: torch.Tensor, with_side_out: bool, keep: bool):
    _check_frame(x)
    for name in ("stages.0.0.weight", "fuse.weight"):
        if not P[name].is_cuda or P[name].dtype != torch.float32:
            raise RuntimeError("OSVOS_VGG parameters must be fp32 tensors on the GPU")
    x = x.contiguous().float()
    N, _, H, W = x.shape
    dev = x.device
    arena = pool.take(N, H, W, dev)
    ap, an = _aligned_ptr(arena)
    w, keep_alive = _weights_struct(P, packs)
    fused = torch.empty((N, 1, H, W), dtype=torch.float32, device=dev)
    outs = [torch.empty((N, 1, H, W), dtype=torch.float32, device=dev) for _ in range(4)] if with_side_out else None
    so = ptr_array4([o.data_ptr() for o in outs]) if with_side_out else None
    idx = dev.index if dev.index is not None else torch.cuda.current_device()
    t0 = ops._pb()
    opts = packs.options
    aux = (pool.aux_stream(idx) if N >= 2 and opts.fwd_aux and opts.two_streams and not packs.flags.forward_one_stream
           else 0)
    pass_flags = VGG_COMPACT_STAGE1 if (packs.flags.compact_stage1 and keep) else 0
    if aux:
        check(lib().fosvos_vgg_forward_streams_flags(pool.ctx(idx), ctypes.byref(w), x.data_ptr(), N, H, W, ap, an,
                                                     fused.data_ptr(), so, torch.cuda.current_stream(idx).cuda_stream, aux,
                                                     pass_flags), "vgg_forward_streams")
    else:
        check(lib().fosvos_vgg_forward_flags(ctypes.byref(w), x.data_ptr(), N, H, W, ap, an, fused.data_ptr(), so, idx,
                                             torch.cuda.current_stream(idx).cuda_stream, pass_flags), "vgg_forward")
    ops._pe(t0, "vgg_forward", 2.0 * 129.114e9 * N * H * W / (480 * 854), 0.0)
    if not keep:
        pool.give(N, H, W, arena)
        arena = None
    return (outs if outs is not None else [None] * 4) + [fused], (arena, x, w, keep_alive, (N, H, W), pass_flags)


def native_backward(P, packs, saved, d_outs, inplace: bool) -> Dict[str, torch.Tensor]:
    arena, x, w, keep_alive, (N, H, W), pass_flags = saved
    dev = x.device
    d_fused = d_outs[4]
    d_so, with_so = _side_grads(d_outs)
    grads: Dict[str, torch.Tensor] = {}
    if d_fused is None and not with_so:
        return grads
    g = VggGrads()
    hold = []

    def slot(name: str) -> int:
        p = P[name]
        if inplace:
            if p.grad is None or p.grad.dtype != torch.float32 or not p.grad.is_contiguous():
                p.grad = torch.zeros_like(p, memory_format=torch.contiguous_format)
            torch.autograd.graph.increment_version(p.grad)
            return p.grad.data_ptr()
        t = torch.empty_like(p, memory_format=torch.contiguous_format)
        grads[name] = t
        return t.data_ptr()

    for c, (wn, bn) in enumerate(_CONV_NAMES):
        g.conv_w[c], g.conv_b[c] = slot(wn), slot(bn)
    for i in range(4):
        g.side_w[i], g.side_b[i] = slot(f"side_prep.{i}.weight"), slot(f"side_prep.{i}.bias")
    g.fuse_w, g.fuse_b = slot("fuse.weight"), slot("fuse.bias")
    dsn_tmp = None
    if with_so:
        dsn_tmp = (torch.zeros((4, 16), dtype=torch.float32, device=dev), torch.zeros((4,), dtype=torch.float32, device=dev))
        g.dsn_w, g.dsn_b = dsn_tmp[0].data_ptr(), dsn_tmp[1].data_ptr()
    flags = packs.flags
    overwrite = inplace and flags.overwrite_grads
    if overwrite and with_so:
        raise RuntimeError("OSVOS_VGG backward: overwrite_grads with side-output gradients (score_dsn accumulates through a scratch)")
    g.accumulate = 1 if inplace and not overwrite else 0
    idx = dev.index if dev.index is not None else torch.cuda.current_device()
    aux = packs.arenas.aux_stream(idx) if packs.options.two_streams else 0
    g.defer_join = 1 if (flags.defer_wgrad_join and inplace and aux) else 0
    g.bucket_events = 1 if flags.publish_grad_buckets else 0
    g.last_pass_of_cycle = 1 if flags.last_pass_of_cycle else 0
    if d_fused is not None:
        d_fused = d_fused.contiguous().float()
        hold.append(d_fused)
    dso = None
    if with_so:
        d_so = [t.contiguous().float() for t in d_so]
        hold += d_so
        dso = ptr_array4([t.data_ptr() for t in d_so])
    ap, an = _aligned_ptr(arena)
    t0 = ops._pb()
    check(lib().fosvos_vgg_backward_flags(packs.arenas.ctx(idx), ctypes.byref(w), ctypes.byref(g), x.data_ptr(), N, H, W, ap, an,
                                          d_fused.data_ptr() if d_fused is not None else None, dso,
                                          torch.cuda.current_stream(idx).cuda_stream, aux or None, pass_flags),
          "vgg_backward")
    ops._pe(t0, "vgg_backward", 2.0 * (2 * 129.114e9 - 0.708e9) * N * H * W / (480 * 854), 0.0)
    if with_so:
        for i in range(4):
            gw, gb = dsn_tmp[0][i].reshape(1, 16, 1, 1), dsn_tmp[1][i:i + 1]
            if inplace:
                for name, val in ((f"score_dsn.{i}.weight", gw), (f"score_dsn.{i}.bias", gb)):
                    p = P[name]
                    if p.grad is None:
                        p.grad = val.clone()
                    else:
                        p.grad.add_(val)
            else:
                grads[f"score_dsn.{i}.weight"], grads[f"score_dsn.{i}.bias"] = gw.clone(), gb.clone()
    del hold, keep_alive
    if g.defer_join:
        packs.arenas.hold(N, H, W, arena, x)
    else:
        packs.arenas.give(N, H, W, arena)
    return grads


class _OSVOSFunction(torch.autograd.Function):

    @staticmethod
    def forward(ctx, packs: PackedWeights, with_side_out: bool, inplace: bool, x: torch.Tensor, *params: torch.Tensor):
        P = dict(zip(PARAM_NAMES, params))
# ... 49 lines not shown
```

### fosvos_amd/fosvos_hip/ops.py

```python
from __future__ import annotations

from typing import List, Optional, Sequence, Tuple

import torch

from . import CONV_OUT_F32, CONV_RELU, check, int_array4, lib, ptr_array4

_BF16 = torch.bfloat16
_F32 = torch.float32


def _need(t: torch.Tensor, dtype, what: str) -> torch.Tensor:
    if not t.is_cuda:
        raise RuntimeError(f"{what}: tensor must live on the GPU (the HIP path has no CPU fallback)")
    if t.dtype != dtype:
        raise TypeError(f"{what}: expected {dtype}, got {t.dtype}")
    if not t.is_contiguous():
        raise ValueError(f"{what}: tensor must be contiguous")
    return t


def _ctx(t: torch.Tensor) -> Tuple[int, int]:
    dev = t.device.index if t.device.index is not None else torch.cuda.current_device()
    return dev, torch.cuda.current_stream(dev).cuda_stream
# ... 278 lines not shown
    L = lib()
    if w_packed.numel() != L.fosvos_packed_weight_elems(co, ci):
        raise ValueError("conv3x3_fwd_pool_codes: packed weight size does not match (Co, Ci)")
    if bias is not None:
        _need(bias, _F32, "conv3x3_fwd_pool_codes bias")
        if bias.numel() != co:
            raise ValueError("conv3x3_fwd_pool_codes: bias size")
    if out is None:
        yp = torch.empty((n, (h + 1) // 2, (wd + 1) // 2, co), dtype=_BF16, device=x.device)
        codes = torch.empty(conv3x3_pool_codes_shape(n, h, wd, co), dtype=torch.int32, device=x.device)
    else:
        yp, codes = out
        _need(yp, _BF16, "conv3x3_fwd_pool_codes pooled output")
        if not (codes.is_cuda and codes.is_contiguous() and codes.dtype == torch.int32):
            raise ValueError("conv3x3_fwd_pool_codes: codes must be a contiguous int32 tensor on the GPU")
        if yp.numel() != n * ((h + 1) // 2) * ((wd + 1) // 2) * co or codes.numel() * 4 != L.fosvos_conv3x3_pool_codes_bytes(n, h, wd, co):
            raise ValueError("conv3x3_fwd_pool_codes: output sizes")
    dev, st = _ctx(x)
    t0 = _pb()
    check(L.fosvos_conv3x3_fwd_pool_codes(x.data_ptr(), w_packed.data_ptr(), _p(bias), yp.data_ptr(), codes.data_ptr(), n, h,
                                          wd, ci, co, CONV_RELU, dev, st), "conv3x3_fwd_pool_codes")
    _pe(t0, "conv3x3_fwd", 2.0 * n * h * wd * 9 * ci * co, n * h * wd * 2 * cx + 2 * 9 * ci * co + yp.numel() * 2 + codes.numel() * 4)
    return yp, codes


def conv3x3_dgrad(dy: torch.Tensor, w_dgrad_packed: torch.Tensor, ci: int, co: int,
                  relu_src: Optional[torch.Tensor] = None, addend: Optional[torch.Tensor] = None,
                  out: Optional[torch.Tensor] = None, relu_bits: Optional[torch.Tensor] = None) -> torch.Tensor:
    _need(dy, _BF16, "conv3x3_dgrad dy"); _need(w_dgrad_packed, _BF16, "conv3x3_dgrad packed weight")
    n, h, wd, cy = dy.shape
    if cy != _ru(co, 32):
        raise ValueError(f"conv3x3_dgrad: dy has {cy} channels, expected {_ru(co, 32)}")
    L = lib()
    if w_dgrad_packed.numel() != L.fosvos_packed_weight_elems(ci, co):
        raise ValueError("conv3x3_dgrad: packed weight size does not match (Ci, Co)")
    shape = (n, h, wd, ci)
    for t, nm in ((relu_src, "relu_src"), (addend, "addend"), (out, "out")):
        if t is not None:
            _need(t, _BF16, f"conv3x3_dgrad {nm}")
            if tuple(t.shape) != shape:
                raise ValueError(f"conv3x3_dgrad: {nm} shape {tuple(t.shape)} != {shape}")
    dx = out if out is not None else torch.empty(shape, dtype=_BF16, device=dy.device)
    ws, wsn = _WS.get(L.fosvos_conv3x3_workspace_bytes(n, h, wd, co, ci), dy.device)
    dev, st = _ctx(dy)
    t0 = _pb()
    if relu_bits is not None:
        if relu_src is not None or relu_bits.dtype != torch.uint8 or tuple(relu_bits.shape) != (n, h, wd, ci // 8) or \
                not relu_bits.is_contiguous() or not relu_bits.is_cuda:
            raise ValueError("conv3x3_dgrad: relu_bits must be a contiguous uint8 [N,H,W,Ci/8] GPU tensor, given instead of relu_src")
        check(L.fosvos_conv3x3_dgrad_bits(dy.data_ptr(), w_dgrad_packed.data_ptr(), relu_bits.data_ptr(), _p(addend),
                                          dx.data_ptr(), n, h, wd, ci, co, ws, wsn, dev, st), "conv3x3_dgrad_bits")
    else:
        check(L.fosvos_conv3x3_dgrad(dy.data_ptr(), w_dgrad_packed.data_ptr(), _p(relu_src), _p(addend), dx.data_ptr(), n, h, wd,
                                     ci, co, ws, wsn, dev, st), "conv3x3_dgrad")
    _pe(t0, "conv3x3_dgrad", 2.0 * n * h * wd * 9 * ci * co,
        n * h * wd * 2 * (cy + ci * (1 + (relu_src is not None) + (addend is not None))) + 2 * 9 * ci * co)
    return dx


def conv3x3_dgrad_unpool(dy: torch.Tensor, w_dgrad_packed: torch.Tensor, ci: int, co: int, x: torch.Tensor,
                         d_pooled: torch.Tensor, out: Optional[torch.Tensor] = None) -> torch.Tensor:
    _need(dy, _BF16, "conv3x3_dgrad_unpool dy"); _need(w_dgrad_packed, _BF16, "conv3x3_dgrad_unpool packed weight")
    _need(x, _BF16, "conv3x3_dgrad_unpool x"); _need(d_pooled, _BF16, "conv3x3_dgrad_unpool d_pooled")
    n, h, wd, cy = dy.shape
    if cy != _ru(co, 32):
        raise ValueError(f"conv3x3_dgrad_unpool: dy has {cy} channels, expected {_ru(co, 32)}")
    L = lib()
    if w_dgrad_packed.numel() != L.fosvos_packed_weight_elems(ci, co):
        raise ValueError("conv3x3_dgrad_unpool: packed weight size does not match (Ci, Co)")
    if tuple(x.shape) != (n, h, wd, ci) or tuple(d_pooled.shape) != (n, (h + 1) // 2, (wd + 1) // 2, ci):
        raise ValueError(f"conv3x3_dgrad_unpool: x {tuple(x.shape)} / d_pooled {tuple(d_pooled.shape)} do not match "
                         f"{(n, h, wd, ci)} and its ceil-mode pooled map")
    if out is not None:
        _need(out, _BF16, "conv3x3_dgrad_unpool out")
        if tuple(out.shape) != (n, h, wd, ci) or out.data_ptr() == x.data_ptr():
            raise ValueError("conv3x3_dgrad_unpool: out must have x's shape and must not alias it")
    dx = out if out is not None else torch.empty((n, h, wd, ci), dtype=_BF16, device=dy.device)
    ws, wsn = _WS.get(L.fosvos_conv3x3_workspace_bytes(n, h, wd, co, ci), dy.device)
    dev, st = _ctx(dy)
    t0 = _pb()
    check(L.fosvos_conv3x3_dgrad_unpool(dy.data_ptr(), w_dgrad_packed.data_ptr(), x.data_ptr(), d_pooled.data_ptr(), dx.data_ptr(),
                                        n, h, wd, ci, co, ws, wsn, dev, st), "conv3x3_dgrad_unpool")
    _pe(t0, "conv3x3_dgrad_unpool", 2.0 * n * h * wd * 9 * ci * co, n * h * wd * 2 * (cy + 2 * ci + ci // 4) + 2 * 9 * ci * co)
    return dx


def conv3x3_wgrad(x: torch.Tensor, dy: torch.Tensor, ci: int, co: int, with_bias: bool = True,
                  dw: Optional[torch.Tensor] = None, db: Optional[torch.Tensor] = None, accumulate: bool = False):
    _need(x, _BF16, "conv3x3_wgrad x"); _need(dy, _BF16, "conv3x3_wgrad dy")
    n, h, wd, cx = x.shape
    if cx != ci or tuple(dy.shape) != (n, h, wd, _ru(co, 32)):
        raise ValueError(f"conv3x3_wgrad: shapes x={tuple(x.shape)} dy={tuple(dy.shape)} do not match Ci={ci} Co={co}")
    L = lib()
    if dw is None:
        if accumulate:
            raise ValueError("conv3x3_wgrad: accumulate needs an existing dw")
        dw = torch.empty((co, ci, 3, 3), dtype=_F32, device=x.device)
    if with_bias and db is None:
        if accumulate:
            raise ValueError("conv3x3_wgrad: accumulate needs an existing db")
        db = torch.empty((co,), dtype=_F32, device=x.device)
    _need(dw, _F32, "conv3x3_wgrad dw")
    ws, wsn = _WS.get(L.fosvos_conv3x3_wgrad_workspace_bytes(n, h, wd, ci, co), x.device)
    dev, st = _ctx(x)
    t0 = _pb()
    check(L.fosvos_conv3x3_wgrad_slabs(x.data_ptr(), dy.data_ptr(), 1 if with_bias else 0, n, h, wd, ci, co, ws, wsn, dev, st),
          "conv3x3_wgrad_slabs")
    _pe(t0, "conv3x3_wgrad", 2.0 * n * h * wd * 9 * ci * co, n * h * wd * 2 * (ci + dy.shape[3]))
    t0 = _pb()
    check(L.fosvos_conv3x3_wgrad_reduce(dw.data_ptr(), _p(db) if with_bias else None, n, h, wd, ci, co,
                                        1 if accumulate else 0, ws, wsn, dev, st), "conv3x3_wgrad_reduce")
    _pe(t0, "wgrad_reduce", 0.0, 4 * 9 * ci * co * 3)
    return dw, (db if with_bias else None)


def conv3x3_wgrad_one_call(x: torch.Tensor, dy: torch.Tensor, ci: int, co: int, with_bias: bool = True):
    _need(x, _BF16, "conv3x3_wgrad x"); _need(dy, _BF16, "conv3x3_wgrad dy")
    n, h, wd, _ = x.shape
    L = lib()
    dw = torch.empty((co, ci, 3, 3), dtype=_F32, device=x.device)
    db = torch.empty((co,), dtype=_F32, device=x.device) if with_bias else None
    ws, wsn = _WS.get(L.fosvos_conv3x3_wgrad_workspace_bytes(n, h, wd, ci, co), x.device)
    dev, st = _ctx(x)
    check(L.fosvos_conv3x3_wgrad(x.data_ptr(), dy.data_ptr(), dw.data_ptr(), _p(db), n, h, wd, ci, co, 0, ws, wsn, dev, st),
          "conv3x3_wgrad")
    return dw, db


def maxpool_fwd(x: torch.Tensor) -> torch.Tensor:
    _need(x, _BF16, "maxpool_fwd")
    n, h, w, c = x.shape
    y = torch.empty((n, (h + 1) // 2, (w + 1) // 2, c), dtype=_BF16, device=x.device)
    dev, st = _ctx(x)
    t0 = _pb()
    check(lib().fosvos_maxpool2x2_ceil_fwd(x.data_ptr(), y.data_ptr(), n, h, w, c, dev, st), "maxpool2x2_ceil_fwd")
    _pe(t0, "maxpool_fwd", 0.0, 2 * (x.numel() + y.numel()))
    return y


def maxpool_bwd(x: torch.Tensor, dy: torch.Tensor, relu_mask: bool = True) -> torch.Tensor:
    _need(x, _BF16, "maxpool_bwd x"); _need(dy, _BF16, "maxpool_bwd dy")
    n, h, w, c = x.shape
    if tuple(dy.shape) != (n, (h + 1) // 2, (w + 1) // 2, c):
        raise ValueError("maxpool_bwd: dy shape mismatch")
    dx = torch.empty_like(x)
    dev, st = _ctx(x)
    t0 = _pb()
    check(lib().fosvos_maxpool2x2_ceil_bwd(x.data_ptr(), dy.data_ptr(), dx.data_ptr(), n, h, w, c, 1 if relu_mask else 0,
                                           dev, st), "maxpool2x2_ceil_bwd")
    _pe(t0, "maxpool_bwd", 0.0, 2 * (2 * x.numel() + dy.numel()))
    return dx


def maxpool_bwd_codes(codes: torch.Tensor, dy: torch.Tensor, h: int, w: int, out: Optional[torch.Tensor] = None) -> torch.Tensor:
    _need(dy, _BF16, "maxpool_bwd_codes dy")
    n, oh, ow, c = dy.shape
    if (oh, ow) != ((h + 1) // 2, (w + 1) // 2) or c % 8:
        raise ValueError("maxpool_bwd_codes: dy shape mismatch")
    if not (codes.is_cuda and codes.is_contiguous() and codes.dtype == torch.int32) or codes.numel() != n * oh * ow * (c // 8):
        raise ValueError("maxpool_bwd_codes: codes must be a contiguous int32 [N, ceil(h/2), ceil(w/2), C/8] tensor on the GPU")
    dx = torch.empty((n, h, w, c), dtype=_BF16, device=dy.device) if out is None else out
    if out is not None:
        _need(out, _BF16, "maxpool_bwd_codes out")
        if out.numel() != n * h * w * c:
            raise ValueError("maxpool_bwd_codes: out size")
    dev, st = _ctx(dy)
# ... 1262 lines not shown
```

### fosvos_amd/networks/osvos_vgg.py

```python
import dataclasses
import os
from copy import deepcopy

import torch
import torch.nn as nn
import torch.nn.modules as modules

from fosvos_hip import engine
from layers.osvos_layers import interp_surgery
from util.logger import get_logger

log = get_logger(__file__)


class OSVOS_VGG(nn.Module):
    def __init__(self, pretrained=1):
        super(OSVOS_VGG, self).__init__()
        lay_list = [[64, 64],
                    ['M', 128, 128],
                    ['M', 256, 256, 256],
                    ['M', 512, 512, 512],
                    ['M', 512, 512, 512]]
        in_channels = [3, 64, 128, 256, 512]

# ... 93 lines not shown
        state = self.__dict__.copy()
        state.pop('_packs', None)
        state.pop('_fosvos_flat_grads', None)
        state['compute_side_outputs'] = True
        state['accumulate_grads_in_place'] = False
        return state

    def __setstate__(self, state):
        self.__dict__.update(state)
        self._packs = engine.PackedWeights()
        self.invalidate_weight_images()

    @staticmethod
    def _make_layers_osvos(cfg, in_channels):
        layers = []
        for v in cfg:
            if v == 'M':
                layers.append(nn.MaxPool2d(kernel_size=2, stride=2, ceil_mode=True))
            else:
                layers.extend([nn.Conv2d(in_channels, v, kernel_size=3, padding=1), nn.ReLU(inplace=True)])
                in_channels = v
        return nn.Sequential(*layers)

    def _initialize_weights(self, pretrained):
        for m in self.modules():
            if isinstance(m, nn.Conv2d):
                m.weight.data.normal_(0, 0.001)
                if m.bias is not None:
                    m.bias.data.zero_()
            elif isinstance(m, nn.ConvTranspose2d):
                m.weight.data.zero_()
                m.weight.data = interp_surgery(m)

        if pretrained == 1:
            self._load_from_pytorch()
        elif pretrained == 2:
            self._load_from_caffe()

    def _load_from_pytorch(self):
        log.info('Loading weights from PyTorch VGG')
        try:
            from torchvision.models import vgg16
        except ImportError as e:
            raise RuntimeError("OSVOS_VGG(pretrained=1) copies torchvision's ImageNet VGG-16, which needs "
                               "torchvision and network access; use pretrained=0 + load_state_dict, or "
                               "pretrained=2 with vgg_hed_caffe.mat") from e
        _vgg = vgg16(pretrained=True)
        src = [m for m in _vgg.features if isinstance(m, nn.Conv2d)]
        dst = [m for stage in self.stages for m in stage if isinstance(m, nn.Conv2d)]
        for d, s in zip(dst, src):
            d.weight = deepcopy(s.weight)
            d.bias = deepcopy(s.bias)

    def _load_from_caffe(self):
        log.info('Loading weights from Caffe VGG')
        import scipy.io
        from config.mypath import Path
        caffe_weights = scipy.io.loadmat(os.path.join(Path.models_dir(), 'vgg_hed_caffe.mat'))
        convs = [m for stage in self.stages for m in stage if isinstance(m, nn.Conv2d)]
        for k, conv in enumerate(convs):
            c_w = torch.from_numpy(caffe_weights['weights'][0][k].transpose())
            c_b = torch.from_numpy(caffe_weights['biases'][0][k][:, 0])
            assert conv.weight.data.shape == c_w.shape
            assert conv.bias.data.shape == c_b.shape
            conv.weight.data = c_w
            conv.bias.data = c_b


def _pass_flag(name):
    def get(self):
        return getattr(self._packs.flags, name)

    def set_(self, value):
        if name == 'defer_wgrad_join' and not value:
            self._packs.arenas.join()
        setattr(self._packs.flags, name, bool(value))

    return property(get, set_, doc='engine.PassFlags.' + name)


for _field in dataclasses.fields(engine.PassFlags):
    setattr(OSVOS_VGG, _field.name, _pass_flag(_field.name))
OSVOS_VGG.compact_stage1 = _pass_flag('compact_stage1')
```

### fosvos_amd/train_offline.py

```python
import timeit
from pathlib import Path
from typing import Optional

import torch
from torch import optim

from config.mypath import Path as P
from fosvos_hip.engine import PassFlags
from fosvos_hip.options import LoopOptions
from layers.osvos_layers import (class_balanced_cross_entropy_loss, class_balanced_cross_entropy_loss_frames_multi,
                                 stage_frames_loss_multi)
from util import gpu_handler, io_helper, experiment_helper, args_helper
from util.logger import get_logger
from util.network_provider import NetworkProvider, provider_mapping
from util.settings import OfflineSettings
import parallel

log = get_logger(__file__)
_hip_cbce = class_balanced_cross_entropy_loss

save_dir_models = Path('models')
save_dir_results = Path('results')
db_root_dir = None
synthetic_size = None
data_parallel = False
resident_train_set = False
microbatch_group = 1


def train_and_test(net_provider: NetworkProvider, settings: OfflineSettings) -> None:
    io_helper.write_settings(save_dir_models, net_provider.name, settings, variant_offline=settings.variant_offline)
    if settings.is_training:
        net_provider.load_network_train()
        shard = (parallel.rank(), parallel.world_size()) if data_parallel else None
        data_loader_train = io_helper.get_data_loader_train(db_root_dir, settings.batch_size_train,
                                                            synthetic=synthetic_size, shard=shard,
                                                            resident_set=resident_train_set)
        data_loader_test = io_helper.get_data_loader_test(db_root_dir, settings.batch_size_test,
                                                          synthetic=synthetic_size)
        optimizer = net_provider.get_optimizer()
        summary_writer = _get_summary_writer()
        _train(net_provider, data_loader_train, data_loader_test, optimizer, summary_writer, settings.start_epoch,
               settings.n_epochs, settings.avg_grad_every_n, settings.snapshot_every_n,
               settings.is_testing_while_training, settings.test_every_n, microbatch_group=microbatch_group)

    if settings.is_testing:
        if not settings.is_training:
            net_provider.load_network_test()
        data_loader = io_helper.get_data_loader_test(db_root_dir, settings.batch_size_test, synthetic=synthetic_size)
        if settings.variant_offline is None:
            save_dir = save_dir_results / net_provider.name / 'offline'
        else:
            save_dir = save_dir_results / net_provider.name / str(settings.variant_offline) / 'offline'
        experiment_helper.test(net_provider, data_loader, save_dir, settings.is_visualizing_results,
                               settings.eval_speeds)


def _get_summary_writer():
    return io_helper.get_summary_writer(save_dir_models, comment='-offline')


def _losses(net, minibatch):
    inputs, gts = gpu_handler.cast_cuda_if_possible([minibatch['image'], minibatch['gt']])
    outputs = net.forward(inputs)
    counts = parallel.batch_label_counts(gts) if data_parallel else None
    return [class_balanced_cross_entropy_loss(o, gts, size_average=False, batch_counts=counts) for o in outputs]


def window_closes(n_window: int, counter_gradient: int, avg_grad_every_n: int, max_window: int, end_of_epoch: bool) -> bool:
    return ((counter_gradient + n_window) % avg_grad_every_n == 0) or n_window >= max_window or end_of_epoch


def plan_passes(shapes, group: int):
    buckets = {}
    for i, shape in enumerate(shapes):
        shape = tuple(int(v) for v in shape)
        alone = shape[0] != 1 or (shape[-2] * shape[-1]) % 4 != 0
        buckets.setdefault(('alone', i) if alone else shape, []).append(i)
    passes = []
    for key, idx in buckets.items():
        if key[0] == 'alone':
            passes.append((idx, False))
        else:
            passes.extend((idx[j:j + group], True) for j in range(0, len(idx), group))
    return passes


def _losses_frames(outputs, gts, map_scale, ones, staged=None):
    k = gts.shape[0]
    if gts.is_cuda and class_balanced_cross_entropy_loss is _hip_cbce:
        return class_balanced_cross_entropy_loss_frames_multi(outputs, gts, map_scale, size_average=False,
                                                              backward_seed=(ones, 1.0), staged=staged), ones[:k]
    losses = torch.stack([torch.stack([class_balanced_cross_entropy_loss(o[i:i + 1], gts[i:i + 1], size_average=False)
                                       for o in outputs]) for i in range(k)])
    return losses, torch.tensor(map_scale, dtype=losses.dtype, device=losses.device).expand(k, -1)


def _train(net_provider: NetworkProvider, data_loader_train, data_loader_test, optimizer: optim.SGD, summary_writer,
           start_epoch: int, n_epochs: int, avg_grad_every_n: int, snapshot_every_n: int,
           is_testing_while_training: bool, test_every_n: int, *, options: Optional[LoopOptions] = None,
           microbatch_group: int = 1, compact_stage1: bool = True) -> dict:
    if options is None:
        options = LoopOptions.from_env()
    microbatch_group = int(microbatch_group)
    if microbatch_group < 1:
        raise ValueError('microbatch_group must be at least 1, got {}'.format(microbatch_group))
    if microbatch_group > 1 and data_parallel:
        raise ValueError('microbatch_group > 1 with data_parallel: that mode splits every BATCH over the ranks with class '
                         'counts of the whole batch; a grouped pass keeps the counts per frame')
    log.info('Start of offline training')
    net = net_provider.network
    flags = getattr(net, 'pass_flags', None) or PassFlags()
    world = parallel.world_size() if data_parallel else 1
    local_accum = avg_grad_every_n
    named = list(net.named_parameters())
    flat = parallel.FlatGrads.attach(net, [p for _, p in named], names=[n for n, _ in named])
    sync = parallel.GradSync(net, flat, options)
    device = next(net.parameters()).device

    n_samples_train = len(data_loader_train)
    loss_train, loss_test, losses_train = [], [], []
    counter_gradient = 0
    n_iters = 0
    n_passes = 0
    max_window = max(microbatch_group, options.group_window)
    ones = torch.ones((microbatch_group, 5), device=device) if microbatch_group > 1 else None
    reserved_frames = getattr(net, 'reserve_arena_frames', None)

    def log_epoch(epoch, running, n_images, start_time):
        if world > 1:
            torch.distributed.all_reduce(running, op=torch.distributed.ReduceOp.SUM)
        vals = (running / n_samples_train).tolist()
        loss_train.append(vals[-1])
        losses_train.append(vals)
        summary_writer.add_scalar('data/total_loss_epoch', vals[-1], epoch)
        log.info('[Epoch: %d, numImages: %5d]' % (epoch, n_images))
        for l in range(len(vals)):
            log.info('Loss %d: %f' % (l, vals[l]))
        log.info('Execution time: ' + str(timeit.default_timer() - start_time))

    def step_if_due():
        nonlocal counter_gradient
        if counter_gradient % local_accum == 0:
            net.join_gradients()
            sync.finish()
            optimizer.step()
            flat.zero()
            counter_gradient = 0

    def run_window(window, epoch, running):
        nonlocal counter_gradient, n_iters, n_passes
        w = 1 - epoch / n_epochs
        map_scale = [w / avg_grad_every_n] * 4 + [1.0 / avg_grad_every_n]
        for idx, batched in plan_passes([mb['image'].shape for mb in window], microbatch_group):
            if not batched:
                losses = _losses(net, window[idx[0]])
                running += torch.stack([l.detach() for l in losses])
                loss = w * sum(losses[:-1]) + losses[-1]
                loss.backward(torch.full_like(loss.detach(), 1.0 / avg_grad_every_n))
            else:
                if len(idx) == 1:
                    inputs, gts = window[idx[0]]['image'], window[idx[0]]['gt']
                else:
                    inputs = torch.cat([window[i]['image'] for i in idx])
                    gts = torch.cat([window[i]['gt'] for i in idx])
                inputs, gts = gpu_handler.cast_cuda_if_possible([inputs, gts])
                staged = None
                if options.stage_loss and gts.is_cuda and class_balanced_cross_entropy_loss is _hip_cbce:
                    staged = stage_frames_loss_multi(gts.contiguous().float(), 5)
                    if staged is not None:
                        gts = staged.label
                outputs = net.forward(inputs)
                losses, seed = _losses_frames(outputs, gts, map_scale, ones, staged)
                losses.backward(seed)
                if staged is not None:
                    staged.finish()
                running += losses.detach().sum(0)
            counter_gradient += len(idx)
            n_iters += len(idx)
            n_passes += 1
        step_if_due()

    time_all_start = timeit.default_timer()
    net.accumulate_grads_in_place = True
    if microbatch_group > 1 and reserved_frames is not None:
        net.reserve_arena_frames = min(microbatch_group, avg_grad_every_n)
    if not options.defer_join:
        net.join_gradients()
    flags.defer_wgrad_join = options.defer_join
    try:
        flags.compact_stage1 = bool(compact_stage1)
        for epoch in range(start_epoch, n_epochs):
            start_time = timeit.default_timer()
            sampler = getattr(data_loader_train, 'sampler', None)
            if hasattr(sampler, 'set_epoch'):
                sampler.set_epoch(epoch)
            running = torch.zeros(5, device=device)
            window = []
            for index, minibatch in enumerate(data_loader_train):
                if microbatch_group > 1:
                    end_of_epoch = index % n_samples_train == n_samples_train - 1
                    window.append(minibatch)
                    if window_closes(len(window), counter_gradient, local_accum, max_window, end_of_epoch):
                        run_window(window, epoch, running)
                        window = []
                    if end_of_epoch:
                        log_epoch(epoch, running, index + 1, start_time)
                    continue
                losses = _losses(net, minibatch)
                running += torch.stack([l.detach() for l in losses])
                loss = (1 - epoch / n_epochs) * sum(losses[:-1]) + losses[-1]

                if index % n_samples_train == n_samples_train - 1:
                    log_epoch(epoch, running, index + 1, start_time)

                last_of_cycle = world > 1 and (counter_gradient + 1) % local_accum == 0
                if last_of_cycle:
                    sync.arm()
                loss.backward(torch.full_like(loss.detach(), 1.0 / avg_grad_every_n))
                if last_of_cycle:
                    sync.begin()
                counter_gradient += 1
                n_iters += 1
                n_passes += 1
                step_if_due()
            if window:
                run_window(window, epoch, running)

            if (epoch % snapshot_every_n) == snapshot_every_n - 1 and epoch != 0 and parallel.rank() == 0:
                net_provider.save_model(epoch)

            if is_testing_while_training and epoch % test_every_n == (test_every_n - 1):
                with torch.no_grad():
                    running_t = torch.zeros(5, device=device)
                    for index, minibatch in enumerate(data_loader_test):
                        running_t += torch.stack(_losses(net, minibatch))
                    vals = (running_t / max(len(data_loader_test), 1)).tolist()
                loss_test.append(vals[-1])
                summary_writer.add_scalar('data/test_loss_epoch', vals[-1], epoch)
                for l in range(len(vals)):
                    log.info('***Testing *** Loss %d: %f' % (l, vals[l]))
        summary_writer.close()
    finally:
        net.join_gradients()
        flags.defer_wgrad_join = False
        flags.compact_stage1 = False
        if microbatch_group > 1 and reserved_frames is not None:
            net.reserve_arena_frames = reserved_frames
    if torch.cuda.is_available():
        torch.cuda.synchronize()
    return {'loss_train': loss_train, 'loss_test': loss_test, 'losses_train': losses_train, 'iterations': n_iters,
            'passes': n_passes, 'seconds': timeit.default_timer() - time_all_start}


def main(argv=None):
    global db_root_dir, synthetic_size, data_parallel, resident_train_set, microbatch_group
    args = args_helper.parse_args(is_online=False, argv=argv)
    if args.network != 'vgg16':
        raise SystemExit('only --network vgg16 is implemented on the HIP path (ResNet family: SURVEY.md §8 f4)')
    data_parallel = bool(args.data_parallel) and parallel.init_distributed()
    gpu_handler.select_gpu(args.gpu_id)
    db_root_dir = P.db_root_dir()
    synthetic_size = (args.height, args.width) if args.synthetic else None
    resident_train_set = bool(args.resident_train_set)
    microbatch_group = args.microbatch_group
    save_dir_models.mkdir(parents=True, exist_ok=True)
    save_dir_results.mkdir(parents=True, exist_ok=True)

    settings = OfflineSettings(is_training=args.is_training, is_testing=args.is_testing, start_epoch=0,
                               n_epochs=args.n_epochs or 240, avg_grad_every_n=args.avg_grad_every_n or 10,
                               snapshot_every_n=40, is_testing_while_training=False, test_every_n=5,
                               batch_size_train=1, batch_size_test=1, is_visualizing_network=False,
                               is_visualizing_results=False, is_loading_vgg_caffe=False,
                               variant_offline=args.variant_offline, eval_speeds=args.eval_speeds)
    provider_class = provider_mapping[('offline', args.network)]
    net_provider = provider_class(args.network, save_dir_models, settings, variant_offline=args.variant_offline)
    if args.synthetic:
        log.warning('--synthetic: starting from OSVOS_VGG(pretrained=0) random init')
        net_provider.load_network_train = lambda: net_provider.init_network(pretrained=0)
    train_and_test(net_provider, settings)


if __name__ == '__main__':
    main()
```

### fosvos_amd/train_online.py

```python
import timeit
from pathlib import Path
from typing import Optional

import numpy as np
import torch
from torch import optim

from config.mypath import Path as P
from fosvos_hip.engine import PassFlags
from fosvos_hip.options import LoopOptions
from layers.osvos_layers import class_balanced_cross_entropy_loss, class_balanced_cross_entropy_loss_frames, stage_frames_loss
from util import gpu_handler, io_helper, experiment_helper, args_helper
from util.logger import get_logger
from util.network_provider import NetworkProvider, provider_mapping
from util.settings import OnlineSettings
import parallel

log = get_logger(__file__)
_hip_cbce = class_balanced_cross_entropy_loss

save_dir_models = Path('models')
save_dir_results = Path('results')
path_stem = 'vgg16/online'
db_root_dir = None
# ... 181 lines not shown

def _losses_per_frame(fused, gts, backward_seed=None, staged=None):
    if fused.is_cuda and class_balanced_cross_entropy_loss is _hip_cbce:
        return class_balanced_cross_entropy_loss_frames(fused, gts, size_average=False, backward_seed=backward_seed,
                                                        staged=staged)
    return torch.stack([class_balanced_cross_entropy_loss(fused[i:i + 1], gts[i:i + 1], size_average=False)
                        for i in range(fused.shape[0])])


class _Landed:

    def query(self):
        return True

    def synchronize(self):
        pass


class _LossLog:

    def __init__(self, ring, n_samples: int, log_every: int, seq_name: str, summary_writer) -> None:
        self.ring = ring
        self.ring_free = list(range(ring.shape[0])) if ring is not None else []
        self.n_samples, self.log_every, self.seq_name, self.summary_writer = n_samples, log_every, seq_name, summary_writer
        self.loss_tr = []
        self.running_host = 0.0
        self.pending = []
        self.window = []

    def flush(self, block: bool) -> None:
        while self.pending:
            items, landed, slots = self.pending[0]
            if block:
                for ev in landed:
                    ev.synchronize()
            elif not all(ev.query() for ev in landed):
                break
            self.pending.pop(0)
            for ep, mb, host_vals, i in items:
                self.running_host += float(host_vals[i])
                if ep % self.log_every == self.log_every - 1:
                    value = self.running_host / self.n_samples
                    self.running_host = 0.0
                    self.loss_tr.append(value)
                    log.info('[Epoch {0}: {1}, numImages: {2}]'.format(self.seq_name, ep + 1, mb + 1))
                    log.info('Loss {0}: {1}'.format(self.seq_name, value))
                    self.summary_writer.add_scalar('data/total_loss_epoch', value, ep)
            self.ring_free.extend(slots)

    def record(self, group, losses) -> None:
        frames = [(g[0], g[1]) for g in group]
        if self.ring is not None:
            if not self.ring_free:
                self.flush(True)
            if not self.ring_free:
                self.window.append((frames, losses.to('cpu'), _Landed(), None))
                return
            slot = self.ring_free.pop()
            host_vals = self.ring[slot, :len(frames)]
            host_vals.copy_(losses, non_blocking=True)
            landed = torch.cuda.Event()
            landed.record()
        else:
            slot, host_vals, landed = None, losses.clone(), _Landed()
        self.window.append((frames, host_vals, landed, slot))

    def close_window(self) -> None:
        if not self.window:
            return
        items = sorted(((ep, mb, host_vals, i) for frames, host_vals, _, _ in self.window
                        for i, (ep, mb) in enumerate(frames)), key=lambda t: (t[0], t[1]))
        slots = [slot for _, _, _, slot in self.window if slot is not None]
        self.pending.append((items, [landed for _, _, landed, _ in self.window], slots))
        self.window.clear()
        self.flush(False)


def _get_summary_writer(seq_name: str):
    return io_helper.get_summary_writer(Path('tensorboard') / path_stem)


def _train(net_provider: NetworkProvider, dataloader, optimizer: optim.SGD, summary_writer, seq_name: str,
           start_epoch: int, n_epochs: int, avg_grad_every_n: int, snapshot_every_n: int, *,
           options: Optional[LoopOptions] = None, compact_stage1: bool = True) -> dict:
    if options is None:
        options = LoopOptions.from_env()
    log.info('Start of Online Training, sequence: ' + seq_name)
    net = net_provider.network
    flags = getattr(net, 'pass_flags', None)
    native = flags is not None and all(callable(getattr(net, f, None)) for f in ('wait_grad_bucket', 'join_gradients'))
    if flags is None:
        flags = PassFlags()
    world = parallel.world_size() if data_parallel else 1
    dp_on = data_parallel and parallel.collectives_on()
    local_accum = parallel.split_accumulation(avg_grad_every_n, world)
    flat = parallel.FlatGrads.attach_module(net)
    sync = parallel.GradSync(net, flat, options)
    on_gpu = flat.flat.is_cuda and native

    early_buckets = [b for b, bid in enumerate(flat.bucket_ids) if bid < parallel.VGG_EARLY_BUCKETS]
    late_buckets = [b for b in range(len(flat.slices)) if b not in early_buckets]
    split_step = (on_gpu and bool(early_buckets) and bool(late_buckets)
                  and getattr(net, 'publishes_grad_buckets', True)
                  and hasattr(optimizer, '_tables') and options.split_step)
    early_params = [p for b in early_buckets for p in flat.bucket_params[b]]
    early_ids = {id(p) for p in early_params}
    late_params = [p for group in optimizer.param_groups for p in group['params'] if id(p) not in early_ids]
    early_prefixes = tuple(pre for b in early_buckets for pre in parallel.VGG_BUCKETS[flat.bucket_ids[b]])

    lazy_zero = on_gpu and options.grad_overwrite
    grads_stale = False
    pass_streams = None
    if flat.flat.is_cuda:
        from fosvos_hip import engine as _engine
        dev_index = flat.flat.device.index if flat.flat.device.index is not None else torch.cuda.current_device()
        _engine.shared_stream(dev_index, "comm")
        if native and options.defer_join and options.pass_streams:
            pass_streams = [None, _engine.shared_stream(dev_index, "pass")]
    counter_gradient = 0
    log_every = max(n_epochs // 20, 1)
    device = next(net.parameters()).device
    max_group = options.microbatch_group
    max_window = max(max_group, options.group_window)
    consts = flat.cache.get(('online', avg_grad_every_n, max_group, str(device)))
    if consts is None:
        consts = flat.cache[('online', avg_grad_every_n, max_group, str(device))] = {
            'inv_avg': torch.ones((), device=device) / avg_grad_every_n,
            'inv_avg_k': torch.full((max_group,), 1.0 / avg_grad_every_n, device=device),
            'ring': torch.empty((64, max_group), dtype=torch.float32).pin_memory() if device.type == 'cuda' else None}
    inv_avg, inv_avg_k = consts['inv_avg'], consts['inv_avg_k']
    loss_log = _LossLog(consts['ring'], len(dataloader), log_every, seq_name, summary_writer)

    def is_snapshot_epoch(epoch: int) -> bool:
        return (epoch % snapshot_every_n) == snapshot_every_n - 1

    side_stream_used = False
    last_pass_on_side = False

    def run_group(group, stream=None) -> None:
        nonlocal counter_gradient, n_iters, side_stream_used, last_pass_on_side
        k = len(group)
        last_pass_on_side = stream is not None
        if stream is not None:
            side_stream_used = True
            with torch.cuda.stream(stream):
                run_pass(group, k)
        else:
            run_pass(group, k)
        counter_gradient += k
        n_iters += k
        close_cycle_if_due()

    def run_pass(group, k) -> None:
        if k == 1:
            inputs, gts = group[0][2]['image'], group[0][2]['gt']
        else:
            inputs = torch.cat([g[2]['image'] for g in group])
            gts = torch.cat([g[2]['gt'] for g in group])
        inputs, gts = gpu_handler.cast_cuda_if_possible([inputs, gts])

        staged = None
        if k > 1 and options.stage_loss and gts.is_cuda and class_balanced_cross_entropy_loss is _hip_cbce:
            staged = stage_frames_loss(gts)

        outputs = net.forward(inputs)

        seeded = outputs[-1].is_cuda and class_balanced_cross_entropy_loss is _hip_cbce
# ... 15 lines not shown
            sync.arm()
        if split_step and closes_cycle:
            flags.publish_grad_buckets = True
        loss.backward(inv_avg if k == 1 else inv_avg_k[:k])
        if last_of_cycle:
            sync.begin()
        if staged is not None:
            staged.finish()
            loss_log.record(group, losses)

    def wait_side_stream() -> None:
        nonlocal side_stream_used
        if side_stream_used:
            torch.cuda.current_stream(device).wait_stream(pass_streams[1])
            side_stream_used = False

    def close_cycle_if_due() -> None:
        nonlocal counter_gradient, grads_stale
        if counter_gradient % local_accum == 0:
            if split_step:
                flags.publish_grad_buckets = False
                if last_pass_on_side:
                    wait_side_stream()
                for b in early_buckets:
                    if dp_on:
                        sync.wait_bucket(b)
                    else:
                        net.wait_grad_bucket(flat.bucket_ids[b])
                optimizer.step(only=early_params, tag='early', zero_grad=not lazy_zero)
                net.prepack_weights(early_prefixes)
                wait_side_stream()
                net.join_gradients()
                sync.finish()
                optimizer.step(only=late_params, tag='late', zero_grad=not lazy_zero)
            else:
                wait_side_stream()
                net.join_gradients()
                sync.finish()
                optimizer.step()
                if not lazy_zero:
                    flat.zero()
            grads_stale = lazy_zero
            counter_gradient = 0

    def run_window(window) -> None:
        nonlocal grads_stale
        buckets = {}
        for item in window:
            shape = tuple(item[2]['image'].shape)
            buckets.setdefault(shape if shape[0] == 1 else ('batch', id(item)), []).append(item)
        groups = [items[i:i + max_group] for items in buckets.values() for i in range(0, len(items), max_group)]
        multi = pass_streams is not None and not dp_on and len(groups) > 1 and max(len(g) for g in groups) <= 2
        if lazy_zero:
            whole_cycle = counter_gradient == 0 and len(groups) == 1 and len(groups[0]) == local_accum
            flags.overwrite_grads = whole_cycle
            if counter_gradient == 0:
                if grads_stale and not whole_cycle:
                    flat.zero()
                grads_stale = False
        if multi:
            net.prepack_weights()
            pass_streams[1].wait_stream(torch.cuda.current_stream(device))
        flags.forward_one_stream = multi
        for i, group in enumerate(groups):
            run_group(group, pass_streams[(len(groups) - 1 - i) % 2] if multi else None)
        if multi:
            wait_side_stream()
        loss_log.close_window()
        epoch, _idx, _mb, end_of_epoch = window[-1]
        if end_of_epoch and is_snapshot_epoch(epoch) and parallel.rank() == 0:
            net_provider.save_model(epoch, sequence=seq_name)

    time_all_start = timeit.default_timer()
    n_iters = 0
    if native:
        net.reserve_arena_frames = min(max_group, avg_grad_every_n)
    net.accumulate_grads_in_place = True
    net.compute_side_outputs = False
    if not options.defer_join:
        net.join_gradients()
    flags.defer_wgrad_join = options.defer_join
    try:
        flags.compact_stage1 = bool(compact_stage1)
        window = []
        for epoch in range(start_epoch, n_epochs):
            n_mb = len(dataloader)
            for minibatch_index, minibatch in enumerate(dataloader):
                end_of_epoch = minibatch_index == n_mb - 1
                window.append((epoch, minibatch_index, minibatch, end_of_epoch))
                closes_cycle = (counter_gradient + len(window)) % local_accum == 0
                if closes_cycle or len(window) >= max_window or (end_of_epoch and is_snapshot_epoch(epoch)):
                    run_window(window)
                    window = []
        if window:
            run_window(window)
    finally:
        net.join_gradients()
        flags.defer_wgrad_join = False
        flags.publish_grad_buckets = False
        if lazy_zero:
            flags.overwrite_grads = False
            if grads_stale:
                flat.zero()
        flags.forward_one_stream = False
        flags.compact_stage1 = False
        net.compute_side_outputs = True
    time_enqueued = timeit.default_timer() - time_all_start
    if torch.cuda.is_available():
        torch.cuda.synchronize()
    loss_log.flush(True)
    time_for_all = timeit.default_timer() - time_all_start
    n_images = len(dataloader)
    log.info('Train {0}: total time {1} sec'.format(seq_name, str(time_for_all)))
    log.info('Train {0}: {1} images'.format(seq_name, str(n_images)))
    log.info('Train {0}: time per sample {1} sec'.format(seq_name, str(time_for_all / max(n_images, 1))))
    return {'loss': loss_log.loss_tr, 'seconds': time_for_all, 'iterations': n_iters, 'seconds_host_enqueue': time_enqueued,
            'comm_timing': sync.timing_summary() if sync.active and sync.timing else None}


def main(argv=None):
    global db_root_dir, synthetic_size, data_parallel, save_dir_models, save_dir_results, score, fast_test, png_fitted, device_decode
    global multi_object, synthetic_objects, clean, adapt
    args = args_helper.parse_args(is_online=True, argv=argv)
    if args.score and args.eval_speeds:
        raise SystemExit('--score needs the PNG-writing test pass; --eval-speeds writes nothing')
    if args.fast_test and args.eval_speeds:
        raise SystemExit('--fast-test is the PNG-writing test pass; --eval-speeds writes nothing')
    score = bool(args.score)
    fast_test = bool(args.fast_test)
    png_fitted = bool(args.png_fitted)
    device_decode = bool(args.device_decode)
    multi_object = bool(args.multi_object)
    clean = None
    if args.clean_min_area is not None or args.clean_largest or args.clean_temporal is not None:
        from fosvos_hip.options import CleanOptions
        clean = CleanOptions(min_area=args.clean_min_area or 0, largest=bool(args.clean_largest),
                             temporal_radius=args.clean_temporal)
    adapt = args.adapt
    synthetic_objects = int(args.objects)
    del scored_sequences[:]
    if args.network != 'vgg16':
        raise SystemExit('only --network vgg16 is implemented on the HIP path (ResNet family: SURVEY.md §8 f4)')
    data_parallel = bool(args.data_parallel) and parallel.init_distributed()
    gpu_handler.select_gpu(args.gpu_id)

    db_root_dir = P.db_root_dir()
    synthetic_size = (args.height, args.width) if args.synthetic else None
    save_dir_models.mkdir(parents=True, exist_ok=True)
    save_dir_results.mkdir(parents=True, exist_ok=True)
    path_input_model = Path(args.parent_model) if args.parent_model else save_dir_models / 'vgg16_epoch-239.pth'
    path_output_model_base = save_dir_models / path_stem
    path_output_model_base.mkdir(parents=True, exist_ok=True)

    settings = OnlineSettings(is_training=args.is_training, is_testing=args.is_testing, start_epoch=0,
                              n_epochs=args.n_epochs or 10000, avg_grad_every_n=args.avg_grad_every_n or 5,
                              snapshot_every_n=args.n_epochs or 10000, is_testing_while_training=False, test_every_n=5,
                              batch_size_train=1, batch_size_test=1, is_visualizing_network=False,
                              is_visualizing_results=False, offline_epoch=240, variant_offline=args.variant_offline,
                              variant_online=args.variant_online, eval_speeds=args.eval_speeds)

    provider_class = provider_mapping[('online', args.network)]

    def make_provider():
        return provider_class(name=args.network, save_dir=(path_input_model, path_output_model_base), settings=settings,
                              variant_offline=args.variant_offline, variant_online=args.variant_online)

    net_provider = make_provider()
    if args.synthetic and not path_input_model.exists():
        from networks.osvos_vgg import OSVOS_VGG
        torch.manual_seed(0)
        if parallel.rank() == 0:
            path_input_model.parent.mkdir(parents=True, exist_ok=True)
            torch.save(OSVOS_VGG(pretrained=0).state_dict(), str(path_input_model))
        if data_parallel:
            torch.distributed.barrier()

    if multi_object:
        if args.sequence_name is not None:
            sequences = [args.sequence_name]
        elif args.synthetic:
            sequences = ['synthetic']
        else:
            from dataloaders.davis_2017 import sequence_names
            sequences = parallel.shard_sequences(sequence_names(db_root_dir, 'val'), args.sequence_group,
                                                 args.sequence_group_size)
        for s in sequences:
            train_and_test_objects(make_provider, s, settings)
        if score and scored_sequences:
# ... 25 lines not shown
```

### include/fosvos_hip.h

```cpp
#ifndef FOSVOS_HIP_H
#define FOSVOS_HIP_H

#include <stddef.h>
#include <stdint.h>

#ifdef __cplusplus
extern "C" {
#endif

#define FOSVOS_ABI_VERSION 33

#define FOSVOS_OK 0
#define FOSVOS_E_SHAPE (-1)
#define FOSVOS_E_ARG (-2)
#define FOSVOS_E_WORKSPACE (-3)
#define FOSVOS_E_HIP (-4)

#define FOSVOS_CONV_RELU 1u
#define FOSVOS_CONV_OUT_F32 2u
#define FOSVOS_CONV_FP32_MATH 4u

int fosvos_abi_version(void);

typedef struct fosvos_profile_record {
// ... 3 lines not shown
    double flops;
} fosvos_profile_record;
int fosvos_profile_start(int device, int max_launches);
int fosvos_profile_stop(int device, fosvos_profile_record *out, int capacity, int *n_out);
const char *fosvos_last_error(void);
const char *fosvos_build_arch(void);

typedef struct fosvos_ctx fosvos_ctx;
int fosvos_ctx_create(int device, fosvos_ctx **ctx_out);
int fosvos_ctx_destroy(fosvos_ctx *ctx);
int fosvos_ctx_device(const fosvos_ctx *ctx);

int fosvos_nchw_f32_to_nhwc_bf16(const float *src, uint16_t *dst, int N, int C, int H, int W, int Cpad,
                                 int device, void *stream);
int fosvos_nhwc_bf16_to_nchw_f32(const uint16_t *src, float *dst, int N, int C, int H, int W, int Cpad,
                                 int device, void *stream);
int fosvos_nhwc_f32_to_nchw_f32(const float *src, float *dst, int N, int C, int H, int W, int device, void *stream);
int fosvos_nchw_f32_to_nhwc_f32(const float *src, float *dst, int N, int C, int H, int W, int device, void *stream);
typedef struct fosvos_vgg_arena_layout_info {
    size_t total;
    int stage_h[5], stage_w[5];
    size_t act[13], gact[13], act_bytes[13];
    size_t pooled[4], gpooled[4], pooled_bytes[4];
    size_t side[4], side_bytes[4];
    size_t dside[4], dside_bytes[4];
    size_t bits0, bits0_bytes;
    size_t ws, ws_bytes, hws, hws_bytes;
    size_t wsa_conv[13], wsa_conv_bytes[13], wsa_side[4], wsa_side_bytes[4];
} fosvos_vgg_arena_layout_info;
int fosvos_vgg_arena_layout(int N, int H, int W, fosvos_vgg_arena_layout_info *out);

int fosvos_pack_conv3x3_weights(const float *w_oihw, int Co, int Ci, uint16_t *w_fwd, uint16_t *w_dgrad,
                                int device, void *stream);
size_t fosvos_packed_weight_elems(int out_ch, int in_ch);

typedef struct fosvos_pack_entry {
    const float *w;
    uint16_t *w_fwd, *w_dgrad;
    int Co, Ci;
} fosvos_pack_entry;
int fosvos_pack_conv3x3_weights_multi(const fosvos_pack_entry *entries, int n, int device, void *stream);

int fosvos_conv3x3_first_fwd(const float *frame, const float *w_oihw, const float *bias, uint16_t *y, uint8_t *relu_bits,
                             int N, int H, int W, int Co, int device, void *stream);
int fosvos_conv3x3_first_plan(int N, int H, int W, int *tiles, int *workgroups);
int fosvos_conv3x3_first_wgrad(const float *frame, const uint16_t *dy, float *dw_oihw, float *dbias, int N, int H,
                               int W, int Co, void *workspace, size_t workspace_bytes, int device, void *stream);
size_t fosvos_conv3x3_first_wgrad_workspace_bytes(int N, int H, int W, int Co);

int fosvos_conv3x3_fwd(const uint16_t *x, const uint16_t *w_packed, const float *bias, void *y, int N, int H, int W,
                       int Ci, int Co, unsigned flags, void *workspace, size_t workspace_bytes, int device,
                       void *stream);

int fosvos_conv3x3_s2_fwd(const uint16_t *x, const uint16_t *w_packed, const float *bias, uint16_t *y, int N, int H, int W,
                          int Ci, int Co, unsigned flags, void *workspace, size_t workspace_bytes, int device, void *stream);
int fosvos_conv3x3_fwd_add(const uint16_t *x, const uint16_t *w_packed, const float *bias, const uint16_t *addend,
                           void *y, int N, int H, int W, int Ci, int Co, unsigned flags, void *workspace,
                           size_t workspace_bytes, int device, void *stream);
int fosvos_conv3x3_fwd_pool(const uint16_t *x, const uint16_t *w_packed, const float *bias, uint16_t *y,
                            uint16_t *y_pool, int N, int H, int W, int Ci, int Co, unsigned flags, void *workspace,
                            size_t workspace_bytes, int device, void *stream);
int fosvos_conv3x3_fwd_pool_codes(const uint16_t *x, const uint16_t *w_packed, const float *bias, uint16_t *y_pool,
                                  uint32_t *codes, int N, int H, int W, int Ci, int Co, unsigned flags, int device,
                                  void *stream);
size_t fosvos_conv3x3_pool_codes_bytes(int N, int H, int W, int C);
size_t fosvos_conv3x3_workspace_bytes(int N, int H, int W, int in_ch, int out_ch);
typedef struct fosvos_conv3x3_plan_info {
    int tile_h, tile_w, tile_co;
    int k_splits;
    int workgroups;
    int persistent;
} fosvos_conv3x3_plan_info;
int fosvos_conv3x3_plan(int N, int H, int W, int in_ch, int out_ch, fosvos_conv3x3_plan_info *out);
int fosvos_conv3x3_fwd_plan(int N, int H, int W, int in_ch, int out_ch, unsigned flags, fosvos_conv3x3_plan_info *out);
int fosvos_conv3x3_dgrad(const uint16_t *dy, const uint16_t *w_dgrad_packed, const uint16_t *relu_src,
                         const uint16_t *addend, uint16_t *dx, int N, int H, int W, int Ci, int Co, void *workspace,
                         size_t workspace_bytes, int device, void *stream);
int fosvos_conv3x3_dgrad_bits(const uint16_t *dy, const uint16_t *w_dgrad_packed, const uint8_t *relu_bits,
                              const uint16_t *addend, uint16_t *dx, int N, int H, int W, int Ci, int Co, void *workspace,
                              size_t workspace_bytes, int device, void *stream);
int fosvos_conv3x3_dgrad_unpool(const uint16_t *dy, const uint16_t *w_dgrad_packed, const uint16_t *x,
                                const uint16_t *d_pooled, uint16_t *dx, int N, int H, int W, int Ci, int Co,
                                void *workspace, size_t workspace_bytes, int device, void *stream);
int fosvos_conv3x3_wgrad(const uint16_t *x, const uint16_t *dy, float *dw_oihw, float *dbias, int N, int H, int W,
                         int Ci, int Co, int accumulate, void *workspace, size_t workspace_bytes, int device,
                         void *stream);
size_t fosvos_conv3x3_wgrad_workspace_bytes(int N, int H, int W, int Ci, int Co);
int fosvos_conv3x3_wgrad_slabs(const uint16_t *x, const uint16_t *dy, int with_bias, int N, int H, int W, int Ci, int Co,
                               void *workspace, size_t workspace_bytes, int device, void *stream);
int fosvos_conv3x3_wgrad_reduce(float *dw_oihw, float *dbias, int N, int H, int W, int Ci, int Co, int accumulate,
                                void *workspace, size_t workspace_bytes, int device, void *stream);

int fosvos_maxpool2x2_ceil_fwd(const uint16_t *x, uint16_t *y, int N, int H, int W, int C, int device, void *stream);
int fosvos_maxpool2x2_ceil_bwd(const uint16_t *x, const uint16_t *dy, uint16_t *dx, int N, int H, int W, int C,
                               int relu_mask, int device, void *stream);
int fosvos_maxpool2x2_ceil_bwd_codes(const uint32_t *codes, const uint16_t *dy, uint16_t *dx, int N, int H, int W, int C,
                                     int device, void *stream);

int fosvos_head_fwd(const float *const side[4], const int hs[4], const int ws[4], const float *const filt[4],
                    const float *const filt1[4], const float *dsn_w , const float *dsn_b ,
                    const float *fuse_w , const float *fuse_b , float *fused,
                    float *const side_out[4] , int N, int H, int W, int filt_uniform, int device,
                    void *stream);
int fosvos_head_bwd(const float *const side[4], const int hs[4], const int ws[4], const float *const filt[4],
                    const float *const filt1[4], const float *dsn_w, const float *fuse_w, const float *d_fused,
                    const float *const d_side_out[4], uint16_t *const d_side[4], float *d_fuse_w, float *d_fuse_b,
                    float *d_dsn_w, float *d_dsn_b, int N, int H, int W, int filt_uniform ,
                    void *workspace, size_t workspace_bytes, int device, void *stream);
size_t fosvos_head_bwd_workspace_bytes(int N, int H, int W);

int fosvos_cbce_loss(const float *logits, const float *label, int64_t numel, int size_average, float grad_scale,
                     float *loss_out, float *grad, void *workspace, size_t workspace_bytes, int device,
                     void *stream);
size_t fosvos_cbce_workspace_bytes(int64_t numel);
int fosvos_cbce_loss_frames(const float *logits, const float *label, int64_t frame_numel, int n_frames, int size_average,
                            float grad_scale, float *loss_out, float *grad, void *workspace, size_t workspace_bytes,
                            int device, void *stream);
#define FOSVOS_CBCE_COUNT 1
#define FOSVOS_CBCE_LOSS 2
#define FOSVOS_CBCE_FINISH 4
int fosvos_cbce_loss_frames_parts(const float *logits, const float *label, int64_t frame_numel, int n_frames,
                                  int size_average, float grad_scale, float *loss_out, float *grad, void *workspace,
                                  size_t workspace_bytes, int parts, int device, void *stream);
#define FOSVOS_CBCE_MAX_MAPS 8
size_t fosvos_cbce_multi_workspace_bytes(int64_t frame_numel, int n_frames, int n_maps);
int fosvos_cbce_loss_frames_multi(const float *const *logits, const float *label, int64_t frame_numel, int n_frames,
                                  int n_maps, int size_average, const float *map_scale, float *loss_out, float *const *grad,
                                  void *workspace, size_t workspace_bytes, int parts, int device, void *stream);
int fosvos_cbce_loss_batch_counts(const float *logits, const float *label, int64_t numel, int size_average,
                                  float grad_scale, const double *batch_counts, float *loss_out, float *grad,
                                  void *workspace, size_t workspace_bytes, int device, void *stream);
size_t fosvos_cbce_void_workspace_bytes(int64_t frame_numel, int n_frames);
int fosvos_cbce_loss_frames_void(const float *logits, const float *label, const uint8_t *void_px, int64_t frame_numel,
                                 int n_frames, int size_average, float grad_scale, float *loss_out, float *grad,
                                 void *workspace, size_t workspace_bytes, int device, void *stream);

#define FOSVOS_SGD_FIRST_STEP 1
#define FOSVOS_SGD_ZERO_GRAD 2
typedef struct fosvos_sgd_entry {
    float *param;
    const float *grad;
    float *momentum_buf;
    int64_t numel;
    float lr;
    float weight_decay;
} fosvos_sgd_entry;
int fosvos_sgd_momentum_step(const fosvos_sgd_entry *table, int n_tensors, int64_t max_numel, float momentum,
                             int first_step, int device, void *stream);

int fosvos_augment_sample(const uint8_t *frame, const uint8_t *mask, int H, int W, int flip, const int32_t *col_taps,
                          const float *col_w, const int32_t *row_taps, const float *row_w, const int32_t *col_near,
                          const int32_t *row_near, int OH, int OW, const float *img_lut, const float *gt_lut, float *image,
                          float *gt, int device, void *stream);

int fosvos_prob_bytes(const float *logits, int N, int H, int W, float *minmax, uint8_t *out, int device, void *stream);
size_t fosvos_jf_workspace_bytes(int N, int H, int W);
int fosvos_jf_counts(const float *logits, const uint8_t *gt, int N, int H, int W, int radius, int32_t *counts,
                     void *workspace, size_t workspace_bytes, int device, void *stream);

size_t fosvos_png_capacity_bytes(int N, int H, int W);
size_t fosvos_png_workspace_bytes(int N, int H, int W, int huffman);
int fosvos_png_encode(const uint8_t *bytes, int N, int H, int W, int huffman, uint8_t *out, size_t capacity, int32_t *lengths,
                      void *workspace, size_t workspace_bytes, int device, void *stream);

#define FOSVOS_MAX_OBJECTS 16
int fosvos_merge_objects(const float *const *logits, int K, int N, int H, int W, uint8_t *labels, int device, void *stream);
// ... 70 lines not shown
int fosvos_conv7x7s2_pool_first_fwd(const float *frame, const float *w_packed, const float *bias, uint16_t *y_pooled, int N,
                                    int H, int W, int Co, int device, void *stream);
int fosvos_maxpool3x3s2_fwd(const uint16_t *x, uint16_t *y, int N, int H, int W, int C, int device, void *stream);
int fosvos_deconv_head_fwd(const float *const side[4], const int hs[4], const int ws[4], const int stride[4],
                           const float *const filt[4], const float *const filt1[4], const float *dsn_w ,
                           const float *dsn_b , const float *fuse_b , float *fused,
                           float *const side_out[4] , int N, int H, int W, int device,
                           void *stream);

typedef struct fosvos_conv2d_desc {
    const void *w_packed;
    const float *bias;
    int Ci, Co, k, stride;
    int kind;
} fosvos_conv2d_desc;
typedef struct fosvos_resnet_block {
    fosvos_conv2d_desc conv[3];
    int n_convs;
    int has_down;
    fosvos_conv2d_desc down;
} fosvos_resnet_block;
typedef struct fosvos_resnet_net {
    const float *first_w;
    const float *first_b;
    int first_co;
    int first_fp32_math;
    int first_unfused;
    int blocks_per_stage[4];
    const fosvos_resnet_block *blocks;
    fosvos_conv2d_desc side[4];
    const float *filt[4];
    const float *filt1[4];
    int stride[4];
    const float *dsn_w, *dsn_b, *fuse_b;
} fosvos_resnet_net;
size_t fosvos_resnet_arena_bytes(const fosvos_resnet_net *net, int N, int H, int W);
int fosvos_resnet_forward(const fosvos_resnet_net *net, const float *frame, int N, int H, int W, void *arena,
                          size_t arena_bytes, float *fused, float *const side_out[4], int device, void *stream,
                          fosvos_ctx *ctx, void *aux_stream);

typedef struct fosvos_vgg_weights {
    const float *conv_w[13];
    const float *conv_b[13];
    const uint16_t *conv_wf[13];
    const uint16_t *conv_wd[13];
    const float *side_b[4];
    const uint16_t *side_wf[4];
    const uint16_t *side_wd[4];
    const float *filt[4];
    const float *filt1[4];
    const float *dsn_w;
    const float *dsn_b;
    const float *fuse_w;
    const float *fuse_b;
    int filt_uniform;
} fosvos_vgg_weights;

typedef struct fosvos_vgg_grads {
    float *conv_w[13];
    float *conv_b[13];
    float *side_w[4];
    float *side_b[4];
    float *dsn_w;
    float *dsn_b;
    float *fuse_w;
    float *fuse_b;
    int accumulate;
    int defer_join;
    int bucket_events;
    int last_pass_of_cycle;
} fosvos_vgg_grads;

size_t fosvos_vgg_arena_bytes(int N, int H, int W);
int fosvos_vgg_forward(const fosvos_vgg_weights *w, const float *frame, int N, int H, int W, void *arena,
                       size_t arena_bytes, float *fused, float *const side_out[4], int device, void *stream);
int fosvos_vgg_forward_streams(fosvos_ctx *ctx, const fosvos_vgg_weights *w, const float *frame, int N, int H, int W,
                               void *arena, size_t arena_bytes, float *fused, float *const side_out[4], void *stream,
                               void *aux_stream);
int fosvos_vgg_backward(fosvos_ctx *ctx, const fosvos_vgg_weights *w, const fosvos_vgg_grads *g, const float *frame, int N,
                        int H, int W, void *arena, size_t arena_bytes, const float *d_fused,
                        const float *const d_side_out[4], void *stream, void *aux_stream);
#define FOSVOS_VGG_COMPACT_STAGE1 1u
int fosvos_vgg_stage1_compact(unsigned flags, int N, int H, int W);
int fosvos_vgg_forward_flags(const fosvos_vgg_weights *w, const float *frame, int N, int H, int W, void *arena,
                             size_t arena_bytes, float *fused, float *const side_out[4], int device, void *stream,
                             unsigned flags);
int fosvos_vgg_forward_streams_flags(fosvos_ctx *ctx, const fosvos_vgg_weights *w, const float *frame, int N, int H, int W,
                                     void *arena, size_t arena_bytes, float *fused, float *const side_out[4], void *stream,
                                     void *aux_stream, unsigned flags);
int fosvos_vgg_backward_flags(fosvos_ctx *ctx, const fosvos_vgg_weights *w, const fosvos_vgg_grads *g, const float *frame,
                              int N, int H, int W, void *arena, size_t arena_bytes, const float *d_fused,
                              const float *const d_side_out[4], void *stream, void *aux_stream, unsigned flags);
int fosvos_vgg_grad_bucket_wait(fosvos_ctx *ctx, int bucket, void *stream);

#ifdef __cplusplus
}
#endif
#endif
```

Before: 1263 frames/s.

## Fuse stage-1 maxpool backward into the conv dgrad epilogue via pool codes

Adds a SCATTER epilogue to the implicit-GEMM conv kernel. The stage-2 first-conv data gradient is routed straight into the dense 2x2 stage-1 map using the saved argmax codes, so the separate maxpool backward kernel can be skipped when compact stage 1 is active. This removes one kernel launch and one read and write of the pooled gradient. In exchange, the epilogue issues four masked 128-bit stores per output vector and split-K is disallowed on this path. The feature is enabled by default in the online and offline training loops.

```diff
diff --git a/fosvos_amd/csrc/conv_igemm.hip b/fosvos_amd/csrc/conv_igemm.hip
--- a/fosvos_amd/csrc/conv_igemm.hip
+++ b/fosvos_amd/csrc/conv_igemm.hip
@@ -20,6 +20,8 @@
     void *y;
     uint16_t *y_pool;
     const uint16_t *unpool_g;
+    const uint32_t *codes;
+    int H1, W1;
     int N, H, W, Cin, Cout, Co_pad;
     int tiles_x, tiles_y;
     unsigned flags;
@@ -109,7 +111,7 @@
     sched_row<MF, NF, 6, NEXT, V>(); sched_row<MF, NF, 7, NEXT, V>();
 }
 
-template <class T, bool OUT_F32, bool UNPOOL = false>
+template <class T, bool OUT_F32, bool UNPOOL = false, bool SCATTER = false>
 __global__ __launch_bounds__(T::NT) __attribute__((amdgpu_waves_per_eu(2, T::WPE))) void k_conv3x3_igemm(const ConvArgs a) {
     extern __shared__ __attribute__((aligned(16))) uint4 smem[];
     uint4 *sA = smem;
@@ -273,7 +275,8 @@
     FOSVOS_STAMP_AT(8)
 
     const int q = lane >> 4, cl = lane & 15;
-    if (a.k_splits > 1) {
+    static_assert(!SCATTER || (!OUT_F32 && !UNPOOL), "the scatter epilogue is a plain bf16 data gradient");
+    if (!SCATTER && a.k_splits > 1) {
         float *po = a.partial + (int64_t)blockIdx.z * a.N * H * W * a.Cout;
 #pragma unroll
         for (int i = 0; i < T::MF; ++i) {
@@ -328,11 +331,18 @@
         const bool ok = it * T::NT + tid < OUT_N && gy < H && o_gx < W;
         voff[it] = ok ? ((gy * W + o_gx) * a.Cout + n0 + o_cg * 8) * 2 : -1;
     }
-    const bool masked = (a.relu_src || a.relu_bits || a.addend) && !(a.flags & kSubsample2);
+    const bool masked = !SCATTER && (a.relu_src || a.relu_bits || a.addend) && !(a.flags & kSubsample2);
     uint4 mk[OUT_IT], ad[OUT_IT];
 #pragma unroll
     for (int it = 0; it < OUT_IT; ++it) mk[it] = ad[it] = make_uint4(0, 0, 0, 0);
-    if constexpr (UNPOOL) {
+    [[maybe_unused]] uint32_t cw[OUT_IT];
+    if constexpr (SCATTER) {
+        auto c_rsrc = __builtin_amdgcn_make_buffer_rsrc(const_cast<uint32_t *>(a.codes + (int64_t)n * H * W * (a.Cout >> 3)), 0,
+                                                        img_bytes >> 2, 0x00020000);
+#pragma unroll
+        for (int it = 0; it < OUT_IT; ++it)
+            cw[it] = __builtin_amdgcn_raw_buffer_load_b32(c_rsrc, voff[it] < 0 ? -1 : voff[it] >> 2, 0, 0);
+    } else if constexpr (UNPOOL) {
         const int OH = (H + 1) >> 1, OW = (W + 1) >> 1;
         auto m_rsrc = __builtin_amdgcn_make_buffer_rsrc(const_cast<uint16_t *>(a.relu_src + (int64_t)n * H * W * a.Cout), 0,
                                                         img_bytes, 0x00020000);
@@ -380,7 +390,7 @@
     float4 bias_r[T::NF];
 #pragma unroll
     for (int j = 0; j < T::NF; ++j)
-        bias_r[j] = a.bias ? *reinterpret_cast<const float4 *>(a.bias + n0 + wn * T::WAVE_N + j * 16 + q * 4)
+        bias_r[j] = (!SCATTER && a.bias) ? *reinterpret_cast<const float4 *>(a.bias + n0 + wn * T::WAVE_N + j * 16 + q * 4)
                            : make_float4(0.f, 0.f, 0.f, 0.f);
     __syncthreads();
     uint16_t *sO = reinterpret_cast<uint16_t *>(smem);
@@ -392,7 +402,7 @@
         for (int i = 0; i < T::MF; ++i) {
             const int pix = wm * T::WAVE_M + i * 16 + cl;
             float v0 = acc[i][j][0] + b.x, v1 = acc[i][j][1] + b.y, v2 = acc[i][j][2] + b.z, v3 = acc[i][j][3] + b.w;
-            if (a.flags & FOSVOS_CONV_RELU) {
+            if (!SCATTER && (a.flags & FOSVOS_CONV_RELU)) {
                 v0 = relu_f(v0); v1 = relu_f(v1); v2 = relu_f(v2); v3 = relu_f(v3);
             }
             *reinterpret_cast<uint2 *>(sO + pix * T::OUT_LD + col) = make_uint2(pack2bf(v0, v1), pack2bf(v2, v3));
@@ -408,6 +418,36 @@
     __syncthreads();
     FOSVOS_STAMP_AT(9)
     const uint16_t *s_vec = sO + o_pix * T::OUT_LD + o_cg * 8;
+    if constexpr (SCATTER) {
+        const int H1 = a.H1, W1 = a.W1;
+        const int px_bytes = a.Cout * 2, row_bytes = W1 * px_bytes;
+        auto d_rsrc = __builtin_amdgcn_make_buffer_rsrc(yo + (int64_t)n * H1 * W1 * a.Cout, 0, H1 * row_bytes, 0x00020000);
+        const bool vx = 2 * o_gx + 1 < W1;
+        const int col_bytes = 2 * o_gx * px_bytes + (n0 + o_cg * 8) * 2;
+#pragma unroll
+        for (int it = 0; it < OUT_IT; ++it) {
+            const int gy = y0 + o_ly + it * ROW_STEP;
+            const bool in = voff[it] >= 0, vy = 2 * gy + 1 < H1;
+            const int o00 = in ? 2 * gy * row_bytes + col_bytes : -1;
+            const int o01 = in && vx ? o00 + px_bytes : -1;
+            const int o10 = in && vy ? o00 + row_bytes : -1;
+            const int o11 = in && vx && vy ? o00 + row_bytes + px_bytes : -1;
+            const uint4 gv = *reinterpret_cast<const uint4 *>(s_vec + it * PIX_STEP * T::OUT_LD);
+            const uint32_t code = cw[it];
+            auto routed = [&](int k) {
+                const uint32_t c = code >> k;
+                return make_uint4(gv.x & ((c & 0x00010001u) * 0xffffu), gv.y & (((c >> 4) & 0x00010001u) * 0xffffu),
+                                  gv.z & (((c >> 8) & 0x00010001u) * 0xffffu), gv.w & (((c >> 12) & 0x00010001u) * 0xffffu));
+            };
+            __builtin_amdgcn_raw_buffer_store_b128(__builtin_bit_cast(u32x4, routed(0)), d_rsrc, o00, 0, 0);
+            __builtin_amdgcn_raw_buffer_store_b128(__builtin_bit_cast(u32x4, routed(1)), d_rsrc, o01, 0, 0);
+            __builtin_amdgcn_raw_buffer_store_b128(__builtin_bit_cast(u32x4, routed(2)), d_rsrc, o10, 0, 0);
+            __builtin_amdgcn_raw_buffer_store_b128(__builtin_bit_cast(u32x4, routed(3)), d_rsrc, o11, 0, 0);
+        }
+        FOSVOS_STAMP_AT(10)
+        FOSVOS_STAMP_RT(12)
+        return;
+    }
     auto y_rsrc = __builtin_amdgcn_make_buffer_rsrc(yo + (int64_t)n * H * W * a.Cout, 0, img_bytes, 0x00020000);
     if constexpr (UNPOOL) {
         static_assert((T::TW & (T::TW - 1)) == 0 && T::TH % 2 == 0, "window partners are pix ^ 1 and pix ^ TW");
@@ -665,7 +705,7 @@
     return p;
 }
 
-template <class T, bool OUT_F32, bool UNPOOL = false>
+template <class T, bool OUT_F32, bool UNPOOL = false, bool SCATTER = false>
 int launch(const ConvArgs &a0, const ConvPlan &plan, hipStream_t st, int in_ch) {
     constexpr int LDS = UNPOOL && 2 * T::LDS_OUT > T::LDS_MAIN ? 2 * T::LDS_OUT : T::LDS_BYTES;
     ConvArgs a = a0;
@@ -683,15 +723,15 @@
         int dev = 0;
         FOSVOS_HIP_CHECK(hipGetDevice(&dev));
         if (dev >= 0 && dev < 64 && !once[dev]) {
-            FOSVOS_HIP_CHECK(hipFuncSetAttribute(reinterpret_cast<const void *>(k_conv3x3_igemm<T, OUT_F32, UNPOOL>),
+            FOSVOS_HIP_CHECK(hipFuncSetAttribute(reinterpret_cast<const void *>(k_conv3x3_igemm<T, OUT_F32, UNPOOL, SCATTER>),
                                                  hipFuncAttributeMaxDynamicSharedMemorySize, LDS));
             once[dev] = true;
         }
     }
     if (g_prof_on) {
         static char name[80];
-        snprintf(name, sizeof(name), "k_conv3x3_igemm<Tile<%d, %d, %d, %d, %d>, %s, %s>", T::TH, T::TW, T::BN, T::WM, T::WN,
-                 OUT_F32 ? "true" : "false", UNPOOL ? "true" : "false");
+        snprintf(name, sizeof(name), "k_conv3x3_igemm<Tile<%d, %d, %d, %d, %d>, %s, %s%s>", T::TH, T::TW, T::BN, T::WM, T::WN,
+                 OUT_F32 ? "true" : "false", UNPOOL ? "true" : "false", SCATTER ? ", true" : "");
         prof_begin(name, st, 2.0 * a.N * a.H * a.W * 9.0 * in_ch * a.Cout);
     }
     {
@@ -710,7 +750,7 @@
     }
     const dim3 grid = a.swizzle ? dim3((unsigned)(tiles * (a.Cout / T::BN)), 1u, (unsigned)plan.k_splits)
                                 : dim3((unsigned)tiles, (unsigned)(a.Cout / T::BN), (unsigned)plan.k_splits);
-    hipLaunchKernelGGL((k_conv3x3_igemm<T, OUT_F32, UNPOOL>), grid, dim3(T::NT), LDS, st, a);
+    hipLaunchKernelGGL((k_conv3x3_igemm<T, OUT_F32, UNPOOL, SCATTER>), grid, dim3(T::NT), LDS, st, a);
     FOSVOS_LAUNCH_CHECK();
     if (plan.k_splits > 1) {
         const int64_t total8 = (a.flags & kSubsample2) ? (int64_t)a.N * ((a.H + 1) >> 1) * ((a.W + 1) >> 1) * (a.Cout / 8)
@@ -746,6 +786,15 @@
         FOSVOS_REQUIRE(workspace && workspace_bytes >= plan.workspace_bytes, FOSVOS_E_WORKSPACE,
                        "conv3x3: split-K needs %zu workspace bytes, got %zu", plan.workspace_bytes, workspace_bytes);
         a.partial = reinterpret_cast<float *>(workspace);
+    }
+    if (a.codes) {
+        FOSVOS_REQUIRE(plan.k_splits == 1, FOSVOS_E_ARG, "conv3x3: the scatter epilogue has no split-K form");
+        switch (plan.tile) {
+            case kBig: return launch<TileBig, false, false, true>(a, plan, st, in_ch);
+            case kSquare: return launch<TileSquare, false, false, true>(a, plan, st, in_ch);
+            case kMid: return launch<TileMid, false, false, true>(a, plan, st, in_ch);
+            default: return fail(FOSVOS_E_ARG, "conv3x3: no scatter epilogue for this tile");
+        }
     }
     if (a.unpool_g) {
         switch (plan.tile) {
@@ -964,6 +1013,33 @@
     return dispatch(a, Co, workspace, workspace_bytes, (hipStream_t)stream);
 }
 
+extern "C" int fosvos_conv3x3_dgrad_unpool_codes(const uint16_t *dy, const uint16_t *w_dgrad_packed, const uint32_t *codes,
+                                                 uint16_t *dx_dense, int N, int H1, int W1, int Ci, int Co, void *workspace,
+                                                 size_t workspace_bytes, int device, void *stream) {
+    FOSVOS_REQUIRE(H1 > 0 && W1 > 0, FOSVOS_E_SHAPE, "conv3x3_dgrad_unpool_codes: bad dense map H1=%d W1=%d", H1, W1);
+    const int H = (H1 + 1) / 2, W = (W1 + 1) / 2;
+    if (int rc = check_common(dy, w_dgrad_packed, dx_dense, N, H, W, Co, Ci, "conv3x3_dgrad_unpool_codes")) return rc;
+    FOSVOS_REQUIRE(codes && ((uintptr_t)codes & 3) == 0, FOSVOS_E_ARG, "conv3x3_dgrad_unpool_codes: null or unaligned codes");
+    FOSVOS_REQUIRE(Ci % 64 == 0, FOSVOS_E_SHAPE, "conv3x3_dgrad_unpool_codes: Ci=%d must be a multiple of 64", Ci);
+    FOSVOS_REQUIRE((int64_t)H1 * W1 * Ci * 2 < 0x7fffffffLL, FOSVOS_E_SHAPE,
+                   "conv3x3_dgrad_unpool_codes: one dense image exceeds 2^31 bytes");
+    {
+        const char *d0 = reinterpret_cast<const char *>(dx_dense), *d1 = d0 + (int64_t)N * H1 * W1 * Ci * 2;
+        const char *y0 = reinterpret_cast<const char *>(dy), *y1 = y0 + (int64_t)N * H * W * roundup(Co, 32) * 2;
+        const char *c0 = reinterpret_cast<const char *>(codes), *c1 = c0 + (int64_t)N * H * W * (Ci / 8) * 4;
+        FOSVOS_REQUIRE((d1 <= y0 || y1 <= d0) && (d1 <= c0 || c1 <= d0), FOSVOS_E_ARG,
+                       "conv3x3_dgrad_unpool_codes: dx_dense overlaps dy or codes");
+    }
+    FOSVOS_ENTER(device);
+    const ConvPlan plan = make_plan(N, H, W, Co, Ci);
+    FOSVOS_REQUIRE(plan.tile == kBig || plan.tile == kSquare || plan.tile == kMid, FOSVOS_E_ARG,
+                   "conv3x3_dgrad_unpool_codes: no scatter epilogue for the tile of N=%d H=%d W=%d", N, H, W);
+    ConvArgs a{};
+    a.x = dy; a.w = w_dgrad_packed; a.codes = codes; a.H1 = H1; a.W1 = W1; a.y = dx_dense;
+    a.N = N; a.H = H; a.W = W; a.Cin = roundup(Co, 32); a.Cout = Ci; a.Co_pad = roundup(Ci, 16); a.flags = kNoSplitK;
+    return dispatch(a, Co, workspace, workspace_bytes, (hipStream_t)stream);
+}
+
 extern "C" int fosvos_conv3x3_dgrad(const uint16_t *dy, const uint16_t *w_dgrad_packed, const uint16_t *relu_src,
                                     const uint16_t *addend, uint16_t *dx, int N, int H, int W, int Ci, int Co,
                                     void *workspace, size_t workspace_bytes, int device, void *stream) {
diff --git a/fosvos_amd/csrc/vgg_net.hip b/fosvos_amd/csrc/vgg_net.hip
--- a/fosvos_amd/csrc/vgg_net.hip
+++ b/fosvos_amd/csrc/vgg_net.hip
@@ -343,8 +343,10 @@
                                          const float *d_fused, const float *const d_side_out[4], void *stream,
                                          void *aux_stream, unsigned flags) {
     FOSVOS_TRY(ctx_check(ctx, "vgg_backward"));
-    FOSVOS_REQUIRE((flags & ~FOSVOS_VGG_COMPACT_STAGE1) == 0, FOSVOS_E_ARG, "vgg_backward: unknown flags 0x%x", flags);
+    FOSVOS_REQUIRE((flags & ~(FOSVOS_VGG_COMPACT_STAGE1 | FOSVOS_VGG_SCATTER_STAGE1)) == 0, FOSVOS_E_ARG,
+                   "vgg_backward: unknown flags 0x%x", flags);
     const bool compact = stage1_compact(flags, N, H, W);
+    const bool scatter = compact && (flags & FOSVOS_VGG_SCATTER_STAGE1) != 0;
     const int device = ctx->device;
     const Arena a = make_arena(N, H, W);
     FOSVOS_TRY(check_net(w, frame, arena, N, H, W, arena_bytes, a, "vgg_backward"));
@@ -443,7 +445,11 @@
                                       base + a.wsa_conv[c], a.wsa_conv_bytes[c], device, sa,
                                       (offload && s == 1) ? &reduce_m : &reduce, tail && s <= tail_stages));
             static const bool bits_on = lab_env_int("FOSVOS_RELU_BITS", 1) != 0;
-            if (c == 1 && bits_on)
+            if (s == 1 && from_pool && scatter)
+                FOSVOS_TRY(fosvos_conv3x3_dgrad_unpool_codes(gact(c), w->conv_wd[c], reinterpret_cast<const uint32_t *>(base + a.act[1]),
+                                                             gact(1), N, a.sh[0], a.sw[0], kCin[c], kCout[c], ws, a.ws_bytes, device,
+                                                             sm));
+            else if (c == 1 && bits_on)
                 FOSVOS_TRY(fosvos_conv3x3_dgrad_bits(gact(c), w->conv_wd[c], reinterpret_cast<const uint8_t *>(base + a.bits0), nullptr,
                                                      dx, N, hh, ww, kCin[c], kCout[c], ws, a.ws_bytes, device, sm));
             else
@@ -456,7 +462,8 @@
                                       base + a.wsa_conv[c], a.wsa_conv_bytes[c], device, sa,
                                       (offload && s == 1) ? &reduce_m : &reduce, tail && s <= tail_stages));
         }
-        if (s == 1 && compact)
+        if (s == 1 && scatter) {
+        } else if (s == 1 && compact)
             FOSVOS_TRY(fosvos_maxpool2x2_ceil_bwd_codes(reinterpret_cast<const uint32_t *>(base + a.act[1]),
                                                         reinterpret_cast<const uint16_t *>(base + a.gpooled[0]), gact(1), N, a.sh[0],
                                                         a.sw[0], kStageCh[0], device, sm));
diff --git a/fosvos_amd/fosvos_hip/__init__.py b/fosvos_amd/fosvos_hip/__init__.py
--- a/fosvos_amd/fosvos_hip/__init__.py
+++ b/fosvos_amd/fosvos_hip/__init__.py
@@ -14,6 +14,7 @@
 CONV_RELU = 1
 CONV_OUT_F32 = 2
 VGG_COMPACT_STAGE1 = 1
+VGG_SCATTER_STAGE1 = 2
 
 
 class FosvosHipError(RuntimeError):
@@ -247,6 +248,8 @@
     "fosvos_conv3x3_pool_codes_bytes": (c_size_t, [c_int, c_int, c_int, c_int]),
     "fosvos_maxpool2x2_ceil_bwd_codes": (c_int, [c_void_p, c_void_p, c_void_p, c_int, c_int, c_int, c_int, c_int, c_void_p]),
     "fosvos_vgg_stage1_compact": (c_int, [c_uint, c_int, c_int, c_int]),
+    "fosvos_conv3x3_dgrad_unpool_codes": (c_int, [c_void_p, c_void_p, c_void_p, c_void_p, c_int, c_int, c_int, c_int, c_int,
+                                                  c_void_p, c_size_t, c_int, c_void_p]),
     "fosvos_vgg_forward_flags": (c_int, [POINTER(VggWeights), c_void_p, c_int, c_int, c_int, c_void_p, c_size_t, c_void_p,
                                          POINTER(c_void_p), c_int, c_void_p, c_uint]),
     "fosvos_vgg_forward_streams_flags": (c_int, [c_void_p, POINTER(VggWeights), c_void_p, c_int, c_int, c_int, c_void_p,
diff --git a/fosvos_amd/fosvos_hip/engine.py b/fosvos_amd/fosvos_hip/engine.py
--- a/fosvos_amd/fosvos_hip/engine.py
+++ b/fosvos_amd/fosvos_hip/engine.py
@@ -7,7 +7,7 @@
 
 import torch
 
-from . import VGG_COMPACT_STAGE1, Context, VggGrads, VggWeights, check, lib, ops, ptr_array4
+from . import VGG_COMPACT_STAGE1, VGG_SCATTER_STAGE1, Context, VggGrads, VggWeights, check, lib, ops, ptr_array4
 from .options import EngineOptions, native_loop_from_env
 
 STAGE_CHANNELS = ((64, 64), (128, 128), (256, 256, 256), (512, 512, 512), (512, 512, 512))
@@ -38,7 +38,7 @@
 
 
 class _PassFlagsSlots:
-    __slots__ = ("_compact_stage1",)
+    __slots__ = ("_compact_stage1", "_scatter_stage1")
 
 
 @dataclass(slots=True)
@@ -57,6 +57,14 @@
     @compact_stage1.setter
     def compact_stage1(self, value: bool) -> None:
         self._compact_stage1 = bool(value)
+
+    @property
+    def scatter_stage1(self) -> bool:
+        return getattr(self, "_scatter_stage1", False)
+
+    @scatter_stage1.setter
+    def scatter_stage1(self, value: bool) -> None:
+        self._scatter_stage1 = bool(value)
 
 
 class PackedWeights:
@@ -481,7 +489,8 @@
     if not keep:
         pool.give(N, H, W, arena)
         arena = None
-    return (outs if outs is not None else [None] * 4) + [fused], (arena, x, w, keep_alive, (N, H, W), pass_flags)
+    bwd_flags = pass_flags | (VGG_SCATTER_STAGE1 if (pass_flags and packs.flags.scatter_stage1) else 0)
+    return (outs if outs is not None else [None] * 4) + [fused], (arena, x, w, keep_alive, (N, H, W), bwd_flags)
 
 
 def native_backward(P, packs, saved, d_outs, inplace: bool) -> Dict[str, torch.Tensor]:
diff --git a/fosvos_amd/fosvos_hip/ops.py b/fosvos_amd/fosvos_hip/ops.py
--- a/fosvos_amd/fosvos_hip/ops.py
+++ b/fosvos_amd/fosvos_hip/ops.py
@@ -384,6 +384,36 @@
     check(L.fosvos_conv3x3_dgrad_unpool(dy.data_ptr(), w_dgrad_packed.data_ptr(), x.data_ptr(), d_pooled.data_ptr(), dx.data_ptr(),
                                         n, h, wd, ci, co, ws, wsn, dev, st), "conv3x3_dgrad_unpool")
     _pe(t0, "conv3x3_dgrad_unpool", 2.0 * n * h * wd * 9 * ci * co, n * h * wd * 2 * (cy + 2 * ci + ci // 4) + 2 * 9 * ci * co)
+    return dx
+
+
+def conv3x3_dgrad_unpool_codes(dy: torch.Tensor, w_dgrad_packed: torch.Tensor, ci: int, co: int, codes: torch.Tensor, h1: int,
+                               w1: int, out: Optional[torch.Tensor] = None) -> torch.Tensor:
+    _need(dy, _BF16, "conv3x3_dgrad_unpool_codes dy"); _need(w_dgrad_packed, _BF16, "conv3x3_dgrad_unpool_codes packed weight")
+    n, h, wd, cy = dy.shape
+    if cy != _ru(co, 32):
+        raise ValueError(f"conv3x3_dgrad_unpool_codes: dy has {cy} channels, expected {_ru(co, 32)}")
+    if (h, wd) != ((h1 + 1) // 2, (w1 + 1) // 2):
+        raise ValueError(f"conv3x3_dgrad_unpool_codes: dy is {h} x {wd}, the pooled map of {h1} x {w1} is "
+                         f"{(h1 + 1) // 2} x {(w1 + 1) // 2}")
+    L = lib()
+    if w_dgrad_packed.numel() != L.fosvos_packed_weight_elems(ci, co):
+        raise ValueError("conv3x3_dgrad_unpool_codes: packed weight size does not match (Ci, Co)")
+    if not (codes.is_cuda and codes.is_contiguous() and codes.dtype == torch.int32) or ci % 8 or \
+            codes.numel() != n * h * wd * (ci // 8):
+        raise ValueError("conv3x3_dgrad_unpool_codes: codes must be a contiguous int32 [N, ceil(h1/2), ceil(w1/2), Ci/8] tensor "
+                         "on the GPU")
+    if out is not None:
+        _need(out, _BF16, "conv3x3_dgrad_unpool_codes out")
+        if out.numel() != n * h1 * w1 * ci:
+            raise ValueError("conv3x3_dgrad_unpool_codes: out size")
+    dx = out if out is not None else torch.empty((n, h1, w1, ci), dtype=_BF16, device=dy.device)
+    dev, st = _ctx(dy)
+    t0 = _pb()
+    check(L.fosvos_conv3x3_dgrad_unpool_codes(dy.data_ptr(), w_dgrad_packed.data_ptr(), codes.data_ptr(), dx.data_ptr(), n, h1, w1,
+                                              ci, co, None, 0, dev, st), "conv3x3_dgrad_unpool_codes")
+    _pe(t0, "conv3x3_dgrad_unpool_codes", 2.0 * n * h * wd * 9 * ci * co,
+        n * h * wd * (2 * cy + ci // 2) + 2 * dx.numel() + 2 * 9 * ci * co)
     return dx
 
 
diff --git a/fosvos_amd/networks/osvos_vgg.py b/fosvos_amd/networks/osvos_vgg.py
--- a/fosvos_amd/networks/osvos_vgg.py
+++ b/fosvos_amd/networks/osvos_vgg.py
@@ -199,3 +199,4 @@
 for _field in dataclasses.fields(engine.PassFlags):
     setattr(OSVOS_VGG, _field.name, _pass_flag(_field.name))
 OSVOS_VGG.compact_stage1 = _pass_flag('compact_stage1')
+OSVOS_VGG.scatter_stage1 = _pass_flag('scatter_stage1')
diff --git a/fosvos_amd/train_offline.py b/fosvos_amd/train_offline.py
--- a/fosvos_amd/train_offline.py
+++ b/fosvos_amd/train_offline.py
@@ -99,7 +99,7 @@
 def _train(net_provider: NetworkProvider, data_loader_train, data_loader_test, optimizer: optim.SGD, summary_writer,
            start_epoch: int, n_epochs: int, avg_grad_every_n: int, snapshot_every_n: int,
            is_testing_while_training: bool, test_every_n: int, *, options: Optional[LoopOptions] = None,
-           microbatch_group: int = 1, compact_stage1: bool = True) -> dict:
+           microbatch_group: int = 1, compact_stage1: bool = True, scatter_stage1: bool = True) -> dict:
     if options is None:
         options = LoopOptions.from_env()
     microbatch_group = int(microbatch_group)
@@ -190,6 +190,7 @@
     flags.defer_wgrad_join = options.defer_join
     try:
         flags.compact_stage1 = bool(compact_stage1)
+        flags.scatter_stage1 = bool(scatter_stage1)
         for epoch in range(start_epoch, n_epochs):
             start_time = timeit.default_timer()
             sampler = getattr(data_loader_train, 'sampler', None)
@@ -245,6 +246,7 @@
         net.join_gradients()
         flags.defer_wgrad_join = False
         flags.compact_stage1 = False
+        flags.scatter_stage1 = False
         if microbatch_group > 1 and reserved_frames is not None:
             net.reserve_arena_frames = reserved_frames
     if torch.cuda.is_available():
diff --git a/fosvos_amd/train_online.py b/fosvos_amd/train_online.py
--- a/fosvos_amd/train_online.py
+++ b/fosvos_amd/train_online.py
@@ -287,7 +287,7 @@
 
 def _train(net_provider: NetworkProvider, dataloader, optimizer: optim.SGD, summary_writer, seq_name: str,
            start_epoch: int, n_epochs: int, avg_grad_every_n: int, snapshot_every_n: int, *,
-           options: Optional[LoopOptions] = None, compact_stage1: bool = True) -> dict:
+           options: Optional[LoopOptions] = None, compact_stage1: bool = True, scatter_stage1: bool = True) -> dict:
     if options is None:
         options = LoopOptions.from_env()
     log.info('Start of Online Training, sequence: ' + seq_name)
@@ -469,6 +469,7 @@
     flags.defer_wgrad_join = options.defer_join
     try:
         flags.compact_stage1 = bool(compact_stage1)
+        flags.scatter_stage1 = bool(scatter_stage1)
         window = []
         for epoch in range(start_epoch, n_epochs):
             n_mb = len(dataloader)
@@ -491,6 +492,7 @@
                 flat.zero()
         flags.forward_one_stream = False
         flags.compact_stage1 = False
+        flags.scatter_stage1 = False
         net.compute_side_outputs = True
     time_enqueued = timeit.default_timer() - time_all_start
     if torch.cuda.is_available():
diff --git a/include/fosvos_hip.h b/include/fosvos_hip.h
--- a/include/fosvos_hip.h
+++ b/include/fosvos_hip.h
@@ -109,6 +109,9 @@
 int fosvos_conv3x3_dgrad_unpool(const uint16_t *dy, const uint16_t *w_dgrad_packed, const uint16_t *x,
                                 const uint16_t *d_pooled, uint16_t *dx, int N, int H, int W, int Ci, int Co,
                                 void *workspace, size_t workspace_bytes, int device, void *stream);
+int fosvos_conv3x3_dgrad_unpool_codes(const uint16_t *dy, const uint16_t *w_dgrad_packed, const uint32_t *codes,
+                                      uint16_t *dx_dense, int N, int H1, int W1, int Ci, int Co, void *workspace,
+                                      size_t workspace_bytes, int device, void *stream);
 int fosvos_conv3x3_wgrad(const uint16_t *x, const uint16_t *dy, float *dw_oihw, float *dbias, int N, int H, int W,
                          int Ci, int Co, int accumulate, void *workspace, size_t workspace_bytes, int device,
                          void *stream);
@@ -345,6 +348,7 @@
                         const float *const d_side_out[4], void *stream, void *aux_stream);
 #define FOSVOS_VGG_COMPACT_STAGE1 1u
 int fosvos_vgg_stage1_compact(unsigned flags, int N, int H, int W);
+#define FOSVOS_VGG_SCATTER_STAGE1 2u
 int fosvos_vgg_forward_flags(const fosvos_vgg_weights *w, const float *frame, int N, int H, int W, void *arena,
                              size_t arena_bytes, float *fused, float *const side_out[4], int device, void *stream,
                              unsigned flags);
```

After: 1263 frames/s. About the same (-0.0%).
